# ai-forever/Kandinsky-2

Hardware: NVIDIA H100
Metric: unet_denoising_steps_per_sec (higher is better)
Workload: dtype f16

## Files before the change

kandinsky-2_b200/csrc/k2_api.cu:

```cuda
#include <stdio.h>
#include <stdlib.h>
#include <string.h>

#include <algorithm>
#include <atomic>
#include <mutex>

#include "../../include/k2b200.h"
#include "k2_internal.h"

namespace k2 {

static thread_local std::string g_err;
static std::atomic<long long> g_launches{0};
static int g_force_bn = 0;
static int g_force_split = 0;
static int g_pdl = 0;


void set_error(const std::string& msg) { g_err = msg; }
int fail(const std::string& msg) {
  g_err = msg;
  return -1;
}
void count_launch(int n) { g_launches.fetch_add(n, std::memory_order_relaxed); }

bool pdl_enabled() { return g_pdl != 0; }
static int g_conv_epi_sets = 1;
static int g_gn_bps = 0;
int gn_apply_blocks_per_sm() { return g_gn_bps; }

int num_sms() {
  static int n = 0;
  if (n == 0) {
    int dev = 0;
    cudaGetDevice(&dev);
    cudaDeviceGetAttribute(&n, cudaDevAttrMultiProcessorCount, dev);
    if (n <= 0) n = 132;
  }
  return n;
}

typedef CUresult (*EncodeTiledFn)(CUtensorMap*, CUtensorMapDataType, cuuint32_t, void*, const cuuint64_t*,
                                  const cuuint64_t*, const cuuint32_t*, const cuuint32_t*,
                                  CUtensorMapInterleave, CUtensorMapSwizzle, CUtensorMapL2promotion,
                                  CUtensorMapFloatOOBfill);

static EncodeTiledFn get_encode_fn() {
  static EncodeTiledFn fn = nullptr;
  static std::once_flag once;
  std::call_once(once, [] {
    void* p = nullptr;
    cudaDriverEntryPointQueryResult qres;
    cudaError_t e = cudaGetDriverEntryPoint("cuTensorMapEncodeTiled", &p, cudaEnableDefault, &qres);
    if (e == cudaSuccess && qres == cudaDriverEntryPointSuccess) fn = reinterpret_cast<EncodeTiledFn>(p);
  });
  return fn;
}

int encode_tmap_f16(CUtensorMap* out, const void* base, int rank, const uint64_t* dims,
                    const uint64_t* strides_bytes, const uint32_t* box) {
  EncodeTiledFn fn = get_encode_fn();
  if (!fn) return fail("cuTensorMapEncodeTiled unavailable (no CUDA driver)");
  cuuint64_t gdim[5];
  cuuint64_t gstr[4];
  cuuint32_t bx[5];
  cuuint32_t es[5];
  for (int i = 0; i < rank; ++i) {
    gdim[i] = dims[i];
    bx[i] = box[i];
    es[i] = 1;
  }
  for (int i = 0; i + 1 < rank; ++i) gstr[i] = strides_bytes[i];
  CUresult r = fn(out, CU_TENSOR_MAP_DATA_TYPE_FLOAT16, static_cast<cuuint32_t>(rank), const_cast<void*>(base),
                  gdim, gstr, bx, es, CU_TENSOR_MAP_INTERLEAVE_NONE, CU_TENSOR_MAP_SWIZZLE_128B,
                  CU_TENSOR_MAP_L2_PROMOTION_L2_256B, CU_TENSOR_MAP_FLOAT_OOB_FILL_NONE);
  if (r != CUDA_SUCCESS) {
    char buf[256];
    snprintf(buf, sizeof buf,
             "cuTensorMapEncodeTiled failed (%d): rank %d dims %llu %llu %llu %llu box %u %u %u %u base %p",
             static_cast<int>(r), rank, (unsigned long long)dims[0], (unsigned long long)(rank > 1 ? dims[1] : 0),
             (unsigned long long)(rank > 2 ? dims[2] : 0), (unsigned long long)(rank > 3 ? dims[3] : 0), box[0],
             rank > 1 ? box[1] : 0, rank > 2 ? box[2] : 0, rank > 3 ? box[3] : 0, base);
    return fail(buf);
  }
  return 0;
}

static void choose_tile(int NB, int H, int W, int& TN, int& TH, int& TW, bool single_image_only = false) {
  long long best_tiles[2] = {-1, -1};
  int bn[2] = {1, 1}, bw[2] = {1, 1}, bh[2] = {1, 1};
  const int wmax = W < 128 ? W : 128;
  for (int tw = 1; tw <= wmax; ++tw) {
    const long long tiles_w = (W + tw - 1) / tw;
    for (int tn = 1; tn <= NB && tn * tw <= 128; ++tn) {
      int thmax = 128 / (tw * tn);
      if (thmax > H) thmax = H;
      if (thmax < 1) continue;
      const long long tiles_h = (H + thmax - 1) / thmax;
      const int th = static_cast<int>((H + tiles_h - 1) / tiles_h);
      const long long tiles = tiles_h * tiles_w * ((NB + tn - 1) / tn);
      for (int k = (tn == 1 ? 0 : 1); k < 2; ++k) {
        bool better = best_tiles[k] < 0 || tiles < best_tiles[k];
        if (!better && tiles == best_tiles[k]) {
          if (tn != bn[k]) {
            better = tn < bn[k];
          } else {
            const int d_new = tw > th ? tw - th : th - tw;
            const int d_old = bw[k] > bh[k] ? bw[k] - bh[k] : bh[k] - bw[k];
            better = (d_new < d_old) || (d_new == d_old && tw > bw[k]);
          }
        }
        if (better) {
          best_tiles[k] = tiles;
          bn[k] = tn;
          bw[k] = tw;
          bh[k] = th;
        }
      }
    }
  }
  const int k = (!single_image_only && best_tiles[1] * 100 <= best_tiles[0] * 85) ? 1 : 0;
  TN = bn[k];
  TW = bw[k];
  TH = bh[k];
}


struct ConvPlan {
  int TN, TH, TW, tiles_w, tiles_h, tiles_n, m_tiles;
  int m_tiles_phase;
  int BN, splits;
  int fuse_stats, row_groups;
  int es;
};

static void plan_conv(int NB, int H, int W, bool any9, int kchunks, int Cout, int out_mode, bool has_workspace,
                      long long workspace_bytes, bool want_gn, ConvPlan& pl, const int* cfg = nullptr, bool up2 = false,
                      bool w_batched = false) {
  const int g_force_bn = (cfg && cfg[0]) ? cfg[0] : k2::g_force_bn;
  const int g_force_split = (cfg && cfg[2]) ? cfg[2] : k2::g_force_split;
  pl.es = (cfg && cfg[3]) ? cfg[3] : k2::g_conv_epi_sets;
  choose_tile(NB, H, W, pl.TN, pl.TH, pl.TW, w_batched);
  pl.tiles_w = (W + pl.TW - 1) / pl.TW;
  pl.tiles_h = (H + pl.TH - 1) / pl.TH;
  pl.tiles_n = (NB + pl.TN - 1) / pl.TN;
  pl.m_tiles = pl.tiles_w * pl.tiles_h * pl.tiles_n;
  pl.m_tiles_phase = pl.m_tiles;

  int BN = g_force_bn;
  int splits = 1;
  const long long M_total = static_cast<long long>(NB) * H * W;
  const bool can_split = !up2 && !w_batched && has_workspace && out_mode == 0 && Cout % 8 == 0;
  auto split_ok = [&](int sp) {
    if (sp == 1) return true;
    const int kps = (kchunks + sp - 1) / sp;
    return can_split && kps >= 8 && (sp - 1) * kps < kchunks &&
           static_cast<long long>(sp) * M_total * Cout * 4 <= workspace_bytes;
  };
  auto model = [&](int bn, int sp) {
    const long long nt = (Cout + bn - 1) / bn;
    const long long units = static_cast<long long>(pl.m_tiles) * nt * sp * (up2 ? 4 : 1);
    const long long slots = num_sms();
    const long long waves = (units + slots - 1) / slots;
    const long long kps = (kchunks + sp - 1) / sp;
    long long cost = waves * (kps * (4LL * bn + 60) + 2000);
    if (sp > 1) cost += 4000 + (static_cast<long long>(sp) + 1) * M_total * Cout * 4 / 1800;
    return cost;
  };
  if (BN == 0) {
    if (Cout <= 16) BN = 16;
    else if (Cout <= 64) BN = 64;
    else if (Cout <= 128) BN = 128;
    else BN = 0;
  }
  {
    const int cand[3] = {256, 192, 128};
    long long best = -1;
    int best_bn = BN ? BN : 256, best_sp = 1;
    for (int ci = 0; ci < 3; ++ci) {
      const int bn = BN ? BN : cand[ci];
      if (BN && ci > 0) break;
      for (int sp = 1; sp <= 8; ++sp) {
        if (g_force_split > 0 && sp != g_force_split) continue;
        if (!split_ok(sp)) continue;
        const long long c = model(bn, sp);
        if (best < 0 || c < best) {
          best = c;
          best_bn = bn;
          best_sp = sp;
        }
      }
    }
    BN = best_bn;
    splits = best_sp;
  }
  pl.BN = BN;
  pl.splits = splits;

  pl.fuse_stats = 0;
  pl.row_groups = 0;
  if (want_gn && out_mode == 0 && Cout % 8 == 0) {
    if (splits == 1 && BN >= 64 && Cout % 64 == 0 && (pl.TN == 1 || pl.TH * pl.TW == 16)) {
      pl.fuse_stats = 1;
      pl.row_groups = ((pl.TN == 1) ? pl.m_tiles : NB * pl.tiles_h * pl.tiles_w) * (up2 ? 4 : 1);
    } else if (splits > 1 && (static_cast<long long>(H) * W) % 16 == 0) {
      pl.fuse_stats = 2;
      pl.row_groups = static_cast<int>(M_total / 16);
    }
  }
}

static void plan_to_info(const ConvPlan& pl, int* info) {
  if (!info) return;
  info[0] = pl.BN; info[1] = 0;
  info[2] = pl.splits; info[3] = pl.m_tiles; info[4] = pl.TN;
  info[5] = pl.fuse_stats; info[6] = pl.row_groups;
}

}

using namespace k2;

extern "C" {

const char* k2_last_error(void) { return g_err.c_str(); }
int k2_version(void) { return 100; }
long long k2_launch_count(void) { return g_launches.load(); }
void k2_reset_launch_count(void) { g_launches.store(0); }
int k2_set_tuning(int key, int value) {
  if (key == 0) {
    g_force_bn = value;
    return 0;
  }
  if (key == 1) {
    g_force_split = value;
    return 0;
  }
  if (key == 2) {
    if (value == 2) return fail("k2_set_tuning: no CTA-pair conv kernel on sm_90");
    return 0;
  }
  if (key == 4) {
    g_pdl = value;
    return 0;
  }
  if (key == 10) {
    g_conv_epi_sets = (value == 2) ? 2 : 1;
    return 0;
  }
  if (key == 11) {
    g_gn_bps = value;
    return 0;
  }
  if (key == 9) {
    return 0;
  }

  return fail("k2_set_tuning: unknown key");
}

int k2_conv_gemm(const K2ConvSrc* srcs, int nsrc, int NB, int H, int W, const void* w_packed, int w_rows,
                 int Ktot, int ldw, int Cout, const float* bias, const void* residual, int ldr, void* out, int ldo,
                 int out_mode, void* workspace, long long workspace_bytes, float* gn_partial, int* info,
                 k2_stream_t stream) {
  return k2_conv_gemm_cfg(srcs, nsrc, NB, H, W, w_packed, w_rows, Ktot, ldw, Cout, bias, residual, ldr, out, ldo, out_mode,
                          workspace, workspace_bytes, gn_partial, info, nullptr, 0, stream);
}

int k2_conv_gemm_cfg(const K2ConvSrc* srcs, int nsrc, int NB, int H, int W, const void* w_packed, int w_rows,
                     int Ktot, int ldw, int Cout, const float* bias, const void* residual, int ldr, void* out, int ldo,
                     int out_mode, void* workspace, long long workspace_bytes, float* gn_partial, int* info,
                     const int* cfg, long long w_batch_stride, k2_stream_t stream) {
  K2_REQUIRE(w_batch_stride >= 0 && w_batch_stride % 8 == 0, "conv_gemm_cfg: w_batch_stride must be a multiple of 8 elements");
  K2_REQUIRE(out_mode == 0 || out_mode == 1, "conv_gemm: out_mode must be 0 (fp16 rows) or 1 (fp32 NCHW)");
  K2_REQUIRE(out_mode == 0 || residual == nullptr, "conv_gemm: out_mode 1 (fp32 NCHW) takes no residual");
  const bool w_batched = w_batch_stride > 0;
  if (cfg) {
    K2_REQUIRE(cfg[0] == 0 || cfg[0] == 16 || cfg[0] == 64 || cfg[0] == 128 || cfg[0] == 192 || cfg[0] == 256,
               "conv_gemm_cfg: N tile must be 0, 16, 64, 128, 192 or 256");
    K2_REQUIRE(cfg[1] >= 0 && cfg[1] <= 2 && cfg[2] >= 0 && cfg[2] <= 8 && cfg[3] >= 0 && cfg[3] <= 2,
               "conv_gemm_cfg: pair mode in 0..2, splits in 0..8, epilogue sets in 0..2");
    K2_REQUIRE(cfg[1] != 2, "conv_gemm_cfg: no CTA-pair conv kernel on sm_90");
  }
  K2_REQUIRE(nsrc >= 1 && nsrc <= 3, "conv_gemm: 1..3 sources");
  K2_REQUIRE((reinterpret_cast<uintptr_t>(gn_partial) & 7) == 0, "conv_gemm: gn_partial must be 8-byte aligned");
  K2_REQUIRE(NB > 0 && H > 0 && W > 0 && Cout > 0, "conv_gemm: bad geometry");
  K2_REQUIRE(w_rows >= Cout, "conv_gemm: w_rows < Cout");
  K2_REQUIRE(Ktot % 64 == 0, "conv_gemm: Ktot must be a multiple of 64");
  if (ldw == 0) ldw = Ktot;
  K2_REQUIRE(ldw >= Ktot && ldw % 8 == 0 && (reinterpret_cast<uintptr_t>(w_packed) & 15) == 0,
             "conv_gemm: weight row stride / alignment");
  ConvGemmParams p;
  memset(&p, 0, sizeof p);
  p.NB = NB;
  p.H = H;
  p.W = W;
  bool any9 = false;
  int kchunks = 0;
  const bool up2 = srcs[0].taps == 4;
  if (up2) {
    K2_REQUIRE(nsrc == 1 && out_mode == 0 && residual == nullptr && H % 2 == 0 && W % 2 == 0,
               "conv_gemm: a taps == 4 source (3x3 conv over its nearest-2x upsampling) must be the only source, with fp16 "
               "output, no residual and even output H, W");
    H /= 2;
    W /= 2;
    p.H = H;
    p.W = W;
  }
  for (int s = 0; s < nsrc; ++s) {
    const K2ConvSrc& src = srcs[s];
    K2_REQUIRE(src.taps == 9 || src.taps == 1 || (s == 0 && src.taps == 4), "conv_gemm: taps must be 9 or 1 (or 4: up2)");
    K2_REQUIRE(src.C > 0 && src.C % 8 == 0 && src.ld % 8 == 0 && src.ld >= src.C, "conv_gemm: bad source C/ld");
    K2_REQUIRE((reinterpret_cast<uintptr_t>(src.ptr) & 15) == 0, "conv_gemm: source not 16B aligned");
    any9 = any9 || src.taps == 9;
    p.seg_taps[s] = src.taps;
    p.seg_kchunks[s] = (src.C + 63) / 64;
    kchunks += src.taps * p.seg_kchunks[s];
  }
  K2_REQUIRE(kchunks * 64 * (up2 ? 4 : 1) == Ktot,
             "conv_gemm: Ktot does not match the sources (taps * ceil(C/64)*64 summed; x4 phases for a taps == 4 source)");
  p.num_k_chunks = kchunks;

  ConvPlan pl;
  plan_conv(NB, H, W, any9 || up2, kchunks, Cout, out_mode, workspace != nullptr, workspace_bytes, gn_partial != nullptr, pl,
            cfg, up2, w_batched);
  K2_REQUIRE(!w_batched || (!up2 && pl.TN == 1), "conv_gemm_cfg: batched weights need single-image tiles");
  p.w_batched = w_batched ? 1 : 0;
  plan_to_info(pl, info);
  p.TN = pl.TN;
  p.TH = pl.TH;
  p.TW = pl.TW;
  p.tiles_w = pl.tiles_w;
  p.tiles_h = pl.tiles_h;
  p.tiles_n = pl.tiles_n;
  p.m_tiles = up2 ? 4 * pl.m_tiles_phase : pl.m_tiles;
  p.m_tiles_phase = pl.m_tiles_phase;
  p.up2 = up2 ? 1 : 0;
  p.a_box_bytes = static_cast<uint32_t>(p.TN * p.TH * p.TW * 128);
  for (int s = 0; s < nsrc; ++s) {
    const K2ConvSrc& src = srcs[s];
    uint64_t dims[4] = {static_cast<uint64_t>(src.C), static_cast<uint64_t>(W), static_cast<uint64_t>(H),
                        static_cast<uint64_t>(NB)};
    uint64_t str[3] = {static_cast<uint64_t>(src.ld) * 2, static_cast<uint64_t>(src.ld) * 2 * W,
                       static_cast<uint64_t>(src.ld) * 2 * W * H};
    uint32_t box[4] = {64, static_cast<uint32_t>(p.TW), static_cast<uint32_t>(p.TH), static_cast<uint32_t>(p.TN)};
    if (encode_tmap_f16(&p.tmA[s], src.ptr, 4, dims, str, box)) return -1;
  }
  const int BN = pl.BN, splits = pl.splits, fuse_stats = pl.fuse_stats;
  p.splits = splits;
  p.k_per_split = (kchunks + splits - 1) / splits;
  p.M_total = static_cast<long long>(NB) * H * W * (up2 ? 4 : 1);
  p.ws = reinterpret_cast<float*>(workspace);
  p.n_tiles = (Cout + BN - 1) / BN;
  p.Cout = Cout;
  {
    uint64_t dims[3] = {static_cast<uint64_t>(Ktot), static_cast<uint64_t>(w_rows), static_cast<uint64_t>(w_batched ? NB : 1)};
    uint64_t str[2] = {static_cast<uint64_t>(ldw) * 2,
                       (w_batched ? static_cast<uint64_t>(w_batch_stride) : static_cast<uint64_t>(ldw) * w_rows) * 2};
    uint32_t box[3] = {64, static_cast<uint32_t>(BN), 1};
    if (encode_tmap_f16(&p.tmB, w_packed, 3, dims, str, box)) return -1;
  }
  p.bias = bias;
  p.residual = reinterpret_cast<const __half*>(residual);
  p.ldr = ldr;
  p.out = out;
  p.ldo = ldo;
  p.out_mode = (splits > 1) ? 2 : out_mode;
  p.gn_part = (fuse_stats == 1) ? reinterpret_cast<float2*>(gn_partial) : nullptr;
  p.gn_mode = (fuse_stats == 1) ? (p.TN == 1 ? 1 : 2) : 0;
  if (out_mode == 0) {
    K2_REQUIRE(ldo % 8 == 0 && (reinterpret_cast<uintptr_t>(out) & 15) == 0, "conv_gemm: out alignment");
    if (residual)
      K2_REQUIRE(ldr % 8 == 0 && (reinterpret_cast<uintptr_t>(residual) & 15) == 0, "conv_gemm: residual alignment");
  }
  int rc = launch_conv_gemm(p, BN, pl.es, static_cast<cudaStream_t>(stream));
  if (rc == 0) g_launches.fetch_add(1, std::memory_order_relaxed);
  if (rc == 0 && splits > 1) {
    rc = launch_splitk_finalize(p.ws, splits, p.M_total, Cout, bias, p.residual, ldr, reinterpret_cast<__half*>(out), ldo,
                                fuse_stats == 2 ? reinterpret_cast<float2*>(gn_partial) : nullptr,
                                static_cast<cudaStream_t>(stream));
    if (rc == 0) g_launches.fetch_add(1, std::memory_order_relaxed);
  }
  return rc;
}

int k2_conv_plan(int NB, int H, int W, int taps, int Ktot, int Cout, int out_mode, long long workspace_bytes,
                 int want_gn_partial, int* info) {
  K2_REQUIRE(NB > 0 && H > 0 && W > 0 && Cout > 0 && info, "conv_plan: bad arguments");
  K2_REQUIRE(Ktot > 0 && Ktot % 64 == 0, "conv_plan: Ktot must be a positive multiple of 64");
  ConvPlan pl;
  plan_conv(NB, H, W, taps == 9, Ktot / 64, Cout, out_mode, workspace_bytes > 0, workspace_bytes, want_gn_partial != 0, pl);
  plan_to_info(pl, info);
  return 0;
}

}
```

kandinsky-2_b200/csrc/k2_common.cuh:

```cuda
#pragma once
#include <cuda.h>
#include <cuda_fp16.h>
#include <cuda_runtime.h>
#include <stdint.h>
#include <stdio.h>

namespace k2 {

__device__ __forceinline__ uint32_t smem_u32(const void* p) {
  return static_cast<uint32_t>(__cvta_generic_to_shared(p));
}

__device__ __forceinline__ uint32_t lane_id() { return threadIdx.x & 31; }

__device__ __forceinline__ bool elect_one() {
  uint32_t pred = 0;
  asm volatile(
      "{\n"
      ".reg .b32 rx;\n"
      ".reg .pred px;\n"
      "elect.sync rx|px, 0xffffffff;\n"
      "selp.b32 %0, 1, 0, px;\n"
      "}\n"
      : "=r"(pred));
  return pred != 0;
}

__device__ __forceinline__ void mbar_init(uint64_t* bar, uint32_t count) {
  asm volatile("mbarrier.init.shared::cta.b64 [%0], %1;" ::"r"(smem_u32(bar)), "r"(count));
}
__device__ __forceinline__ void fence_barrier_init() {
  asm volatile("fence.mbarrier_init.release.cluster;" ::: "memory");
}
__device__ __forceinline__ void mbar_arrive_expect_tx(uint64_t* bar, uint32_t bytes) {
  asm volatile("mbarrier.arrive.expect_tx.shared::cta.b64 _, [%0], %1;" ::"r"(smem_u32(bar)),
               "r"(bytes)
               : "memory");
}
__device__ __forceinline__ void mbar_arrive(uint64_t* bar) {
  asm volatile("mbarrier.arrive.shared::cta.b64 _, [%0];" ::"r"(smem_u32(bar)) : "memory");
}
__device__ __forceinline__ bool mbar_try_wait(uint64_t* bar, uint32_t parity) {
  uint32_t ok;
  asm volatile(
      "{\n"
      ".reg .pred p;\n"
      "mbarrier.try_wait.parity.shared::cta.b64 p, [%1], %2;\n"
      "selp.b32 %0, 1, 0, p;\n"
      "}\n"
      : "=r"(ok)
      : "r"(smem_u32(bar)), "r"(parity)
      : "memory");
  return ok != 0;
}
__device__ __forceinline__ void mbar_wait(uint64_t* bar, uint32_t parity) {
  if (mbar_try_wait(bar, parity)) return;
  long long t0 = clock64();
  while (!mbar_try_wait(bar, parity)) {
    if (clock64() - t0 > 4000000000LL) {
      printf("k2b200: mbarrier wait timeout (block %d,%d,%d thread %d)\n", blockIdx.x, blockIdx.y,
             blockIdx.z, threadIdx.x);
      __trap();
    }
  }
}

__device__ __forceinline__ void mbar_wait_lean(uint64_t* bar, uint32_t parity) {
  if (mbar_try_wait(bar, parity)) return;
  long long t0 = clock64();
  while (!mbar_try_wait(bar, parity)) {
    if (clock64() - t0 > 4000000000LL) __trap();
  }
}

__device__ __forceinline__ void fence_proxy_async_smem() {
  asm volatile("fence.proxy.async.shared::cta;" ::: "memory");
}

__device__ __forceinline__ void tma_prefetch_desc(const CUtensorMap* tm) {
  asm volatile("prefetch.tensormap [%0];" ::"l"(reinterpret_cast<uint64_t>(tm)) : "memory");
}
__device__ __forceinline__ void tma_load_2d(void* dst, const CUtensorMap* tm, uint64_t* bar, int c0,
                                            int c1) {
  asm volatile(
      "cp.async.bulk.tensor.2d.shared::cluster.global.mbarrier::complete_tx::bytes [%0], [%1, {%3, "
      "%4}], [%2];"
      ::"r"(smem_u32(dst)),
      "l"(reinterpret_cast<uint64_t>(tm)), "r"(smem_u32(bar)), "r"(c0), "r"(c1)
      : "memory");
}
__device__ __forceinline__ void tma_load_3d(void* dst, const CUtensorMap* tm, uint64_t* bar, int c0,
                                            int c1, int c2) {
  asm volatile(
      "cp.async.bulk.tensor.3d.shared::cluster.global.mbarrier::complete_tx::bytes [%0], [%1, {%3, "
      "%4, %5}], [%2];"
      ::"r"(smem_u32(dst)),
      "l"(reinterpret_cast<uint64_t>(tm)), "r"(smem_u32(bar)), "r"(c0), "r"(c1), "r"(c2)
      : "memory");
}
__device__ __forceinline__ void tma_load_4d(void* dst, const CUtensorMap* tm, uint64_t* bar, int c0,
                                            int c1, int c2, int c3) {
  asm volatile(
      "cp.async.bulk.tensor.4d.shared::cluster.global.mbarrier::complete_tx::bytes [%0], [%1, {%3, "
      "%4, %5, %6}], [%2];"
      ::"r"(smem_u32(dst)),
      "l"(reinterpret_cast<uint64_t>(tm)), "r"(smem_u32(bar)), "r"(c0), "r"(c1), "r"(c2), "r"(c3)
      : "memory");
}

__device__ __forceinline__ uint64_t make_wgmma_desc(uint32_t smem_addr) {
  uint64_t d = 0;
  d |= static_cast<uint64_t>((smem_addr & 0x3FFFF) >> 4);
  d |= static_cast<uint64_t>(1) << 16;
  d |= static_cast<uint64_t>(1024 >> 4) << 32;
  d |= static_cast<uint64_t>(1) << 62;
  return d;
}
__device__ __forceinline__ void wgmma_fence() { asm volatile("wgmma.fence.sync.aligned;" ::: "memory"); }
__device__ __forceinline__ void wgmma_commit() { asm volatile("wgmma.commit_group.sync.aligned;" ::: "memory"); }
template <int N>
__device__ __forceinline__ void wgmma_wait() {
  asm volatile("wgmma.wait_group.sync.aligned %0;" ::"n"(N) : "memory");
}
__device__ __forceinline__ void wgmma_m64n16k16(float (&d)[8], uint64_t adesc, uint64_t bdesc, uint32_t accumulate) {
  asm volatile(
      "{\n"
      ".reg .pred p;\n"
      "setp.ne.b32 p, %10, 0;\n"
      "wgmma.mma_async.sync.aligned.m64n16k16.f32.f16.f16 "
      "{%0, %1, %2, %3, %4, %5, %6, %7}, %8, %9, p, 1, 1, 0, 0;\n"
      "}\n"
      : "+f"(d[0]), "+f"(d[1]), "+f"(d[2]), "+f"(d[3]), "+f"(d[4]), "+f"(d[5]), "+f"(d[6]), "+f"(d[7])
      : "l"(adesc), "l"(bdesc), "r"(accumulate));
}

__device__ __forceinline__ void wgmma_m64n64k16(float (&d)[32], uint64_t adesc, uint64_t bdesc, uint32_t accumulate) {
  asm volatile(
      "{\n"
      ".reg .pred p;\n"
      "setp.ne.b32 p, %34, 0;\n"
      "wgmma.mma_async.sync.aligned.m64n64k16.f32.f16.f16 "
      "{%0, %1, %2, %3, %4, %5, %6, %7, %8, %9, %10, %11, %12, %13, %14, %15, %16, %17, %18, %19, %20, %21, %22, %23, %24, %25, %26, %27, %28, %29, %30, %31}, %32, %33, p, 1, 1, 0, 0;\n"
      "}\n"
      : "+f"(d[0]), "+f"(d[1]), "+f"(d[2]), "+f"(d[3]), "+f"(d[4]), "+f"(d[5]), "+f"(d[6]), "+f"(d[7]), "+f"(d[8]), "+f"(d[9]), "+f"(d[10]), "+f"(d[11]), "+f"(d[12]), "+f"(d[13]), "+f"(d[14]), "+f"(d[15]), "+f"(d[16]), "+f"(d[17]), "+f"(d[18]), "+f"(d[19]), "+f"(d[20]), "+f"(d[21]), "+f"(d[22]), "+f"(d[23]), "+f"(d[24]), "+f"(d[25]), "+f"(d[26]), "+f"(d[27]), "+f"(d[28]), "+f"(d[29]), "+f"(d[30]), "+f"(d[31])
      : "l"(adesc), "l"(bdesc), "r"(accumulate));
}

#define K2_WGMMA_D8(o)                                                                                                  \
  "+f"(d[(o)]), "+f"(d[(o) + 1]), "+f"(d[(o) + 2]), "+f"(d[(o) + 3]), "+f"(d[(o) + 4]), "+f"(d[(o) + 5]), "+f"(d[(o) + 6]), \
      "+f"(d[(o) + 7])
#define K2_WGMMA_D32(o) K2_WGMMA_D8(o), K2_WGMMA_D8((o) + 8), K2_WGMMA_D8((o) + 16), K2_WGMMA_D8((o) + 24)

__device__ __forceinline__ void wgmma_m64n128k16(float (&d)[64], uint64_t adesc, uint64_t bdesc, uint32_t accumulate) {
  asm volatile(
      "{\n"
      ".reg .pred p;\n"
      "setp.ne.b32 p, %66, 0;\n"
      "wgmma.mma_async.sync.aligned.m64n128k16.f32.f16.f16 {"
      "%0, %1, %2, %3, %4, %5, %6, %7, %8, %9, %10, %11, %12, %13, %14, %15, "
      "%16, %17, %18, %19, %20, %21, %22, %23, %24, %25, %26, %27, %28, %29, %30, %31, "
      "%32, %33, %34, %35, %36, %37, %38, %39, %40, %41, %42, %43, %44, %45, %46, %47, "
      "%48, %49, %50, %51, %52, %53, %54, %55, %56, %57, %58, %59, %60, %61, %62, %63"
      "}, %64, %65, p, 1, 1, 0, 0;\n"
      "}\n"
      : K2_WGMMA_D32(0), K2_WGMMA_D32(32)
      : "l"(adesc), "l"(bdesc), "r"(accumulate));
}

__device__ __forceinline__ void wgmma_m64n192k16(float (&d)[96], uint64_t adesc, uint64_t bdesc, uint32_t accumulate) {
  asm volatile(
      "{\n"
      ".reg .pred p;\n"
      "setp.ne.b32 p, %98, 0;\n"
      "wgmma.mma_async.sync.aligned.m64n192k16.f32.f16.f16 {"
      "%0, %1, %2, %3, %4, %5, %6, %7, %8, %9, %10, %11, %12, %13, %14, %15, "
      "%16, %17, %18, %19, %20, %21, %22, %23, %24, %25, %26, %27, %28, %29, %30, %31, "
      "%32, %33, %34, %35, %36, %37, %38, %39, %40, %41, %42, %43, %44, %45, %46, %47, "
      "%48, %49, %50, %51, %52, %53, %54, %55, %56, %57, %58, %59, %60, %61, %62, %63, "
      "%64, %65, %66, %67, %68, %69, %70, %71, %72, %73, %74, %75, %76, %77, %78, %79, "
      "%80, %81, %82, %83, %84, %85, %86, %87, %88, %89, %90, %91, %92, %93, %94, %95"
      "}, %96, %97, p, 1, 1, 0, 0;\n"
      "}\n"
      : K2_WGMMA_D32(0), K2_WGMMA_D32(32), K2_WGMMA_D32(64)
      : "l"(adesc), "l"(bdesc), "r"(accumulate));
}

__device__ __forceinline__ void wgmma_m64n256k16(float (&d)[128], uint64_t adesc, uint64_t bdesc, uint32_t accumulate) {
  asm volatile(
      "{\n"
      ".reg .pred p;\n"
      "setp.ne.b32 p, %130, 0;\n"
      "wgmma.mma_async.sync.aligned.m64n256k16.f32.f16.f16 {"
      "%0, %1, %2, %3, %4, %5, %6, %7, %8, %9, %10, %11, %12, %13, %14, %15, "
      "%16, %17, %18, %19, %20, %21, %22, %23, %24, %25, %26, %27, %28, %29, %30, %31, "
      "%32, %33, %34, %35, %36, %37, %38, %39, %40, %41, %42, %43, %44, %45, %46, %47, "
      "%48, %49, %50, %51, %52, %53, %54, %55, %56, %57, %58, %59, %60, %61, %62, %63, "
      "%64, %65, %66, %67, %68, %69, %70, %71, %72, %73, %74, %75, %76, %77, %78, %79, "
      "%80, %81, %82, %83, %84, %85, %86, %87, %88, %89, %90, %91, %92, %93, %94, %95, "
      "%96, %97, %98, %99, %100, %101, %102, %103, %104, %105, %106, %107, %108, %109, %110, %111, "
      "%112, %113, %114, %115, %116, %117, %118, %119, %120, %121, %122, %123, %124, %125, %126, %127"
      "}, %128, %129, p, 1, 1, 0, 0;\n"
      "}\n"
      : K2_WGMMA_D32(0), K2_WGMMA_D32(32), K2_WGMMA_D32(64), K2_WGMMA_D32(96)
      : "l"(adesc), "l"(bdesc), "r"(accumulate));
}
__device__ __forceinline__ uint64_t make_wgmma_desc_mn(uint32_t smem_addr) {
  uint64_t d = 0;
  d |= static_cast<uint64_t>((smem_addr & 0x3FFFF) >> 4);
  d |= static_cast<uint64_t>(1) << 16;
  d |= static_cast<uint64_t>(1024 >> 4) << 32;
  d |= static_cast<uint64_t>(1) << 62;
  return d;
}

__device__ __forceinline__ void wgmma_m64n64k16_rs_tb(float (&d)[32], const uint32_t (&a)[4], uint64_t bdesc) {
  asm volatile(
      "{\n"
      "wgmma.mma_async.sync.aligned.m64n64k16.f32.f16.f16 {"
      "%0, %1, %2, %3, %4, %5, %6, %7, %8, %9, %10, %11, %12, %13, %14, %15, "
      "%16, %17, %18, %19, %20, %21, %22, %23, %24, %25, %26, %27, %28, %29, %30, %31"
      "}, {%32, %33, %34, %35}, %36, 1, 1, 1, 1;\n"
      "}\n"
      : K2_WGMMA_D32(0)
      : "r"(a[0]), "r"(a[1]), "r"(a[2]), "r"(a[3]), "l"(bdesc));
}
#undef K2_WGMMA_D32
#undef K2_WGMMA_D8

__device__ __forceinline__ void reg_fence(float& r) { asm volatile("" : "+f"(r)::"memory"); }

template <int R>
__device__ __forceinline__ void setmaxnreg_dec() {
  asm volatile("setmaxnreg.dec.sync.aligned.u32 %0;" ::"n"(R));
}
template <int R>
__device__ __forceinline__ void setmaxnreg_inc() {
  asm volatile("setmaxnreg.inc.sync.aligned.u32 %0;" ::"n"(R));
}

__device__ __forceinline__ void mma_16816(float (&d)[4], const uint32_t (&a)[4], uint32_t b0, uint32_t b1) {
  asm volatile(
      "mma.sync.aligned.m16n8k16.row.col.f32.f16.f16.f32 {%0, %1, %2, %3}, {%4, %5, %6, %7}, {%8, %9}, "
      "{%0, %1, %2, %3};"
      : "+f"(d[0]), "+f"(d[1]), "+f"(d[2]), "+f"(d[3])
      : "r"(a[0]), "r"(a[1]), "r"(a[2]), "r"(a[3]), "r"(b0), "r"(b1));
}
__device__ __forceinline__ void ldmatrix_x4(uint32_t (&r)[4], uint32_t saddr) {
  asm volatile("ldmatrix.sync.aligned.m8n8.x4.shared.b16 {%0, %1, %2, %3}, [%4];"
               : "=r"(r[0]), "=r"(r[1]), "=r"(r[2]), "=r"(r[3])
               : "r"(saddr));
}
__device__ __forceinline__ void ldmatrix_x4_trans(uint32_t (&r)[4], uint32_t saddr) {
  asm volatile("ldmatrix.sync.aligned.m8n8.x4.trans.shared.b16 {%0, %1, %2, %3}, [%4];"
               : "=r"(r[0]), "=r"(r[1]), "=r"(r[2]), "=r"(r[3])
               : "r"(saddr));
}
__device__ __forceinline__ void cp_async_16(uint32_t saddr, const void* gptr, int src_bytes) {
  asm volatile("cp.async.cg.shared.global [%0], [%1], 16, %2;" ::"r"(saddr), "l"(gptr), "r"(src_bytes) : "memory");
}
__device__ __forceinline__ void cp_async_commit() { asm volatile("cp.async.commit_group;" ::: "memory"); }
template <int N>
__device__ __forceinline__ void cp_async_wait() {
  asm volatile("cp.async.wait_group %0;" ::"n"(N) : "memory");
}

__device__ __forceinline__ void sts_v4(uint32_t saddr, uint32_t a, uint32_t b, uint32_t c, uint32_t d) {
  asm volatile("st.shared.v4.b32 [%0], {%1, %2, %3, %4};" ::"r"(saddr), "r"(a), "r"(b), "r"(c), "r"(d) : "memory");
}
__device__ __forceinline__ uint4 lds_v4(uint32_t saddr) {
  uint4 v;
  asm volatile("ld.shared.v4.b32 {%0, %1, %2, %3}, [%4];" : "=r"(v.x), "=r"(v.y), "=r"(v.z), "=r"(v.w) : "r"(saddr) : "memory");
  return v;
}
__device__ __forceinline__ uint32_t lds_u32(uint32_t saddr) {
  uint32_t v;
  asm volatile("ld.shared.b32 %0, [%1];" : "=r"(v) : "r"(saddr) : "memory");
  return v;
}
__device__ __forceinline__ void named_bar_sync(int id, int count) {
  asm volatile("bar.sync %0, %1;" ::"r"(id), "r"(count) : "memory");
}
__device__ __forceinline__ void named_bar_arrive(int id, int count) {
  asm volatile("bar.arrive %0, %1;" ::"r"(id), "r"(count) : "memory");
}
__device__ __forceinline__ void pdl_wait() { asm volatile("griddepcontrol.wait;" ::: "memory"); }
__device__ __forceinline__ void pdl_launch() { asm volatile("griddepcontrol.launch_dependents;" ::: "memory"); }

__device__ __forceinline__ float silu_f(float x) {
  float e, r;
  asm("ex2.approx.ftz.f32 %0, %1;" : "=f"(e) : "f"(-1.44269504088896341f * x));
  asm("rcp.approx.ftz.f32 %0, %1;" : "=f"(r) : "f"(1.f + e));
  return x * r;
}

}
```

kandinsky-2_b200/csrc/k2_conv_gemm.cu:

```cuda
#include <stdio.h>

#include "k2_common.cuh"
#include "k2_internal.h"

namespace k2 {

namespace {

constexpr int BM = 128;
constexpr int BK = 64;
constexpr int A_STAGE_BYTES = BM * BK * 2;
constexpr int ACC_PAD = 4;

constexpr int EPI_STAGE_FLOATS = 32 * 33;
constexpr int EPI_BYTES = 4 * EPI_STAGE_FLOATS * 4 + 4 * 256 * 4;
constexpr int SMEM_LIMIT = 227 * 1024;

template <int BN, int ES>
struct Cfg {
  static constexpr int B_STAGE_BYTES = BN * BK * 2;
  static constexpr int STAGE_BYTES = A_STAGE_BYTES + B_STAGE_BYTES;
  static constexpr int BNC = (BN < 64) ? BN : (ES == 2 ? 128 : 64);
  static_assert(ES == 1 || BN % 128 == 0, "two epilogue sets need N tiles of 128 or 256");
  static constexpr int ACC_BYTES = BM * (BNC + ACC_PAD) * 4;
  static constexpr int BAR_BYTES = 256;
  static constexpr int FIXED = ACC_BYTES + ES * EPI_BYTES + BAR_BYTES + 1024;
  static constexpr int STAGES = (SMEM_LIMIT - FIXED) / STAGE_BYTES > 6 ? 6 : (SMEM_LIMIT - FIXED) / STAGE_BYTES;
  static constexpr int SMEM_BYTES = STAGES * STAGE_BYTES + FIXED;
  static_assert(STAGES >= 2, "conv_gemm: shared memory does not hold two pipeline stages");
};

__device__ __forceinline__ void decode_m_tile(const ConvGemmParams& p, int m_idx, int& n0, int& y0,
                                              int& x0, int& phase) {
  phase = 0;
  if (p.up2) {
    phase = m_idx / p.m_tiles_phase;
    m_idx -= phase * p.m_tiles_phase;
  }
  int tw_i = m_idx % p.tiles_w;
  int t = m_idx / p.tiles_w;
  int th_i = t % p.tiles_h;
  int tn_i = t / p.tiles_h;
  x0 = tw_i * p.TW;
  y0 = th_i * p.TH;
  n0 = tn_i * p.TN;
}

template <int N>
__device__ __forceinline__ void acc_ld(const float* src, uint32_t (&r)[N]) {
#pragma unroll
  for (int v = 0; v < N / 4; ++v) {
    const float4 t = *reinterpret_cast<const float4*>(src + 4 * v);
    r[4 * v] = __float_as_uint(t.x);
    r[4 * v + 1] = __float_as_uint(t.y);
    r[4 * v + 2] = __float_as_uint(t.z);
    r[4 * v + 3] = __float_as_uint(t.w);
  }
}

template <int BN, int ES>
__device__ __forceinline__ void epilogue_tile(const ConvGemmParams& p, const float* acc, int ew, int lane, int n0, int y0,
                                              int x0, int cbase, int split, int m_idx, float* stat_smem, int es_arg,
                                              int phase) {
  const int es = (ES == 1) ? 0 : es_arg;
  const int row = ew * 32 + lane;
  const int thw = p.TH * p.TW;
  constexpr int CH = (BN >= 32) ? 32 : 16;
  const float* arow = acc + row * (BN + ACC_PAD);
      const int tn = row / thw;
      const int rem = row - tn * thw;
      const int th = rem / p.TW;
      const int tw = rem - th * p.TW;
      const int n = n0 + tn, y = y0 + th, x = x0 + tw;
      const bool valid = (tn < p.TN) && (n < p.NB) && (y < p.H) && (x < p.W);
      const long long out_row = p.up2 ? (static_cast<long long>(n) * (2 * p.H) + (2 * y + (phase >> 1))) * (2 * p.W) + (2 * x + (phase & 1))
                                      : (static_cast<long long>(n) * p.H + y) * p.W + x;
      const int m_in = p.up2 ? m_idx - phase * p.m_tiles_phase : m_idx;
      auto part_index = [&](long long base) { return p.up2 ? base * 4 + phase : base; };
      if constexpr (BN % 64 == 0) {
        if ((p.out_mode == 0 && p.Cout % 64 == 0) || (p.out_mode == 2 && p.Cout % 32 == 0)) {
          const uint32_t stage = smem_u32(stat_smem + (es * 4 + ew) * EPI_STAGE_FLOATS);
          float* bsm = stat_smem + 4 * ES * EPI_STAGE_FLOATS + (es * 4 + ew) * 256;
          const int my_pix = valid ? static_cast<int>(out_row) : -1;
          const int sub = lane >> 3, piece = lane & 7;
          int pix[8];
#pragma unroll
          for (int i = 0; i < 8; ++i) pix[i] = __shfl_sync(0xffffffffu, my_pix, i * 4 + sub);
          const uint32_t own = stage + lane * 128;
          if (p.out_mode == 2) {
            float* wsb = p.ws + static_cast<long long>(split) * p.M_total * p.Cout;
#pragma unroll 1
            for (int j = 0; j < BN / 32; ++j) {
              const int col0 = cbase + j * 32;
              if (col0 >= p.Cout) break;
              if constexpr (ES > 1) {
                if ((j % ES) != es) continue;
              }
              uint32_t r[32];
              acc_ld(arow + j * 32, r);
#pragma unroll
              for (int v = 0; v < 8; ++v)
                sts_v4(own + ((v ^ (lane & 7)) << 4), r[v * 4], r[v * 4 + 1], r[v * 4 + 2], r[v * 4 + 3]);
              __syncwarp();
#pragma unroll
              for (int i = 0; i < 8; ++i) {
                const int rr = i * 4 + sub;
                const uint4 v4 = lds_v4(stage + rr * 128 + ((piece ^ (rr & 7)) << 4));
                if (pix[i] >= 0)
                  *reinterpret_cast<uint4*>(wsb + static_cast<long long>(pix[i]) * p.Cout + col0 + piece * 4) = v4;
              }
              __syncwarp();
            }
            return;
          }
          constexpr int NP = BN / 64;
          if (p.bias) {
#pragma unroll
            for (int c = lane; c < BN; c += 32) bsm[c] = (cbase + c < p.Cout) ? __ldg(p.bias + cbase + c) : 0.f;
            __syncwarp();
          }
          __half* outb = reinterpret_cast<__half*>(p.out);
          float4 st[NP];
          uint4 rpre[8];
          auto load_res = [&](int jp) {
            const int c0 = cbase + jp * 64;
#pragma unroll
            for (int i = 0; i < 8; ++i) {
              rpre[i] = make_uint4(0u, 0u, 0u, 0u);
              if (pix[i] >= 0 && c0 < p.Cout)
                rpre[i] = *reinterpret_cast<const uint4*>(p.residual + static_cast<long long>(pix[i]) * p.ldr + c0 + piece * 8);
            }
          };
          if constexpr (ES == 1) {
            if (p.residual) load_res(0);
          }
#pragma unroll
          for (int jp = 0; jp < NP; ++jp) {
            const int col0 = cbase + jp * 64;
            st[jp] = make_float4(0.f, 0.f, 0.f, 0.f);
            if (col0 < p.Cout && (ES == 1 || (jp % ES) == es)) {
              if constexpr (ES > 1) {
                if (p.residual) load_res(jp);
              }
              if (p.residual) {
#pragma unroll
                for (int i = 0; i < 8; ++i) {
                  const int rr = i * 4 + sub;
                  sts_v4(stage + rr * 128 + ((piece ^ (rr & 7)) << 4), rpre[i].x, rpre[i].y, rpre[i].z, rpre[i].w);
                }
                __syncwarp();
              }
              if constexpr (ES == 1) {
                if (p.residual && jp + 1 < NP) load_res(jp + 1);
              }
#pragma unroll
              for (int v = 0; v < 8; ++v) {
                uint32_t r[8];
                acc_ld(arow + jp * 64 + v * 8, r);
                float f[8];
#pragma unroll
                for (int e = 0; e < 8; ++e) f[e] = __uint_as_float(r[e]);
                if (p.bias) {
                  const float4 b0 = *reinterpret_cast<const float4*>(bsm + jp * 64 + v * 8);
                  const float4 b1 = *reinterpret_cast<const float4*>(bsm + jp * 64 + v * 8 + 4);
                  f[0] += b0.x; f[1] += b0.y; f[2] += b0.z; f[3] += b0.w;
                  f[4] += b1.x; f[5] += b1.y; f[6] += b1.z; f[7] += b1.w;
                }
                const uint32_t slot = own + ((v ^ (lane & 7)) << 4);
                if (p.residual) {
                  const uint4 rv = lds_v4(slot);
                  const __half2* rh = reinterpret_cast<const __half2*>(&rv);
#pragma unroll
                  for (int e = 0; e < 4; ++e) {
                    const float2 t = __half22float2(rh[e]);
                    f[2 * e] += t.x;
                    f[2 * e + 1] += t.y;
                  }
                }
                uint32_t o[4];
#pragma unroll
                for (int e = 0; e < 4; ++e) {
                  const __half2 hh = __floats2half2_rn(f[2 * e], f[2 * e + 1]);
                  o[e] = valid ? *reinterpret_cast<const uint32_t*>(&hh) : 0u;
                }
                sts_v4(slot, o[0], o[1], o[2], o[3]);
              }
              __syncwarp();
#pragma unroll
              for (int i = 0; i < 8; ++i) {
                const int rr = i * 4 + sub;
                const uint4 v4 = lds_v4(stage + rr * 128 + ((piece ^ (rr & 7)) << 4));
                if (pix[i] >= 0)
                  *reinterpret_cast<uint4*>(outb + static_cast<long long>(pix[i]) * p.ldo + col0 + piece * 8) = v4;
              }
              if (p.gn_part) {
                float4 h0 = make_float4(0.f, 0.f, 0.f, 0.f), h1 = make_float4(0.f, 0.f, 0.f, 0.f);
#pragma unroll
                for (int rr = 0; rr < 32; ++rr) {
                  const uint32_t w = lds_u32(stage + rr * 128 + (((lane >> 2) ^ (rr & 7)) << 4) + ((lane & 3) << 2));
                  const float2 t = __half22float2(*reinterpret_cast<const __half2*>(&w));
                  float4& hacc = (rr < 16) ? h0 : h1;
                  hacc.x += t.x;
                  hacc.y = fmaf(t.x, t.x, hacc.y);
                  hacc.z += t.y;
                  hacc.w = fmaf(t.y, t.y, hacc.w);
                }
                if (p.gn_mode == 2) {
                  const int per = p.tiles_h * p.tiles_w;
                  const int sp = m_in % per;
                  const int img = n0 + 2 * ew;
                  if (2 * ew < p.TN && img < p.NB)
                    *reinterpret_cast<float4*>(p.gn_part + part_index(static_cast<long long>(img) * per + sp) * p.Cout + col0 + 2 * lane) = h0;
                  if (2 * ew + 1 < p.TN && img + 1 < p.NB)
                    *reinterpret_cast<float4*>(p.gn_part + part_index(static_cast<long long>(img + 1) * per + sp) * p.Cout + col0 + 2 * lane) = h1;
                } else {
                  st[jp] = make_float4(h0.x + h1.x, h0.y + h1.y, h0.z + h1.z, h0.w + h1.w);
                }
              }
              __syncwarp();
            }
          }
          if (p.gn_part && p.gn_mode == 1) {
            if constexpr (ES == 1) {
              float4* mine = reinterpret_cast<float4*>(stat_smem + ew * EPI_STAGE_FLOATS);
#pragma unroll
              for (int jp = 0; jp < NP; ++jp) mine[jp * 32 + lane] = st[jp];
              named_bar_sync(1, 128);
              if (ew < NP) {
                const int col0 = cbase + ew * 64;
                if (col0 < p.Cout) {
                  float4 acc = make_float4(0.f, 0.f, 0.f, 0.f);
#pragma unroll
                  for (int w = 0; w < 4; ++w) {
                    const float4 t = reinterpret_cast<const float4*>(stat_smem + w * EPI_STAGE_FLOATS)[ew * 32 + lane];
                    acc.x += t.x; acc.y += t.y; acc.z += t.z; acc.w += t.w;
                  }
                  *reinterpret_cast<float4*>(p.gn_part + part_index(m_in) * p.Cout + col0 + 2 * lane) = acc;
                }
              }
              named_bar_sync(1, 128);
            } else {
              float4* mine = reinterpret_cast<float4*>(stat_smem + (es * 4 + ew) * EPI_STAGE_FLOATS);
#pragma unroll
              for (int jp = 0; jp < NP; ++jp) mine[jp * 32 + lane] = st[jp];
              named_bar_sync(1 + es, 128);
              const int jp_f = es + ew * ES;
              if (jp_f < NP) {
                const int col0 = cbase + jp_f * 64;
                if (col0 < p.Cout) {
                  float4 acc = make_float4(0.f, 0.f, 0.f, 0.f);
#pragma unroll
                  for (int w = 0; w < 4; ++w) {
                    const float4 t =
                        reinterpret_cast<const float4*>(stat_smem + (es * 4 + w) * EPI_STAGE_FLOATS)[jp_f * 32 + lane];
                    acc.x += t.x; acc.y += t.y; acc.z += t.z; acc.w += t.w;
                  }
                  *reinterpret_cast<float4*>(p.gn_part + part_index(m_in) * p.Cout + col0 + 2 * lane) = acc;
                }
              }
              named_bar_sync(1 + es, 128);
            }
          }
          return;
        }
      }
#pragma unroll 1
      for (int j = 0; j < BN / CH; ++j) {
        uint32_t r[CH];
        acc_ld(arow + j * CH, r);
        const int col0 = cbase + j * CH;
        if (valid && col0 < p.Cout) {
          if (p.out_mode == 2) {
            float* w = p.ws + (static_cast<long long>(split) * p.M_total + out_row) * p.Cout + col0;
            if (col0 + CH <= p.Cout) {
#pragma unroll
              for (int v = 0; v < CH / 4; ++v)
                *reinterpret_cast<uint4*>(w + v * 4) = make_uint4(r[v * 4], r[v * 4 + 1], r[v * 4 + 2], r[v * 4 + 3]);
            } else {
#pragma unroll
              for (int e = 0; e < CH; ++e)
                if (col0 + e < p.Cout) w[e] = __uint_as_float(r[e]);
            }
          } else if (p.out_mode == 0) {
            __half* orow = reinterpret_cast<__half*>(p.out) + out_row * p.ldo + col0;
            const __half* rrow = p.residual ? p.residual + out_row * p.ldr + col0 : nullptr;
            if (col0 + CH <= p.Cout) {
#pragma unroll
              for (int v = 0; v < CH / 8; ++v) {
                float f[8];
#pragma unroll
                for (int e = 0; e < 8; ++e) {
                  f[e] = __uint_as_float(r[v * 8 + e]);
                  if (p.bias) f[e] += __ldg(p.bias + col0 + v * 8 + e);
                }
                if (rrow) {
                  uint4 rv = *reinterpret_cast<const uint4*>(rrow + v * 8);
                  const __half2* rh = reinterpret_cast<const __half2*>(&rv);
#pragma unroll
                  for (int e = 0; e < 4; ++e) {
                    float2 t = __half22float2(rh[e]);
                    f[2 * e] += t.x;
                    f[2 * e + 1] += t.y;
                  }
                }
                uint4 ov;
                __half2* oh = reinterpret_cast<__half2*>(&ov);
#pragma unroll
                for (int e = 0; e < 4; ++e) oh[e] = __floats2half2_rn(f[2 * e], f[2 * e + 1]);
                *reinterpret_cast<uint4*>(orow + v * 8) = ov;
              }
            } else {
#pragma unroll
              for (int e = 0; e < CH; ++e) {
                if (col0 + e < p.Cout) {
                  float f = __uint_as_float(r[e]);
                  if (p.bias) f += __ldg(p.bias + col0 + e);
                  if (rrow) f += __half2float(rrow[e]);
                  orow[e] = __float2half_rn(f);
                }
              }
            }
          } else {
            float* o = reinterpret_cast<float*>(p.out);
#pragma unroll
            for (int e = 0; e < CH; ++e) {
              if (col0 + e < p.Cout) {
                float f = __uint_as_float(r[e]);
                if (p.bias) f += __ldg(p.bias + col0 + e);
                o[((static_cast<long long>(n) * p.Cout + (col0 + e)) * p.H + y) * p.W + x] = f;
              }
            }
          }
        }
      }
}


template <int BN, int ES>
__global__ void __launch_bounds__(384, 1) conv_gemm_kernel(const __grid_constant__ ConvGemmParams p) {
  using C = Cfg<BN, ES>;
  constexpr int BNC = C::BNC;
  constexpr int NA = BN / 2;
  extern __shared__ uint8_t smem_raw[];
  uint8_t* smem = reinterpret_cast<uint8_t*>((reinterpret_cast<uintptr_t>(smem_raw) + 1023) &
                                             ~static_cast<uintptr_t>(1023));
  float* acc_smem = reinterpret_cast<float*>(smem + C::STAGES * C::STAGE_BYTES);
  float* stat_smem = reinterpret_cast<float*>(smem + C::STAGES * C::STAGE_BYTES + C::ACC_BYTES);
  uint64_t* full_bar = reinterpret_cast<uint64_t*>(smem + C::STAGES * C::STAGE_BYTES + C::ACC_BYTES + ES * EPI_BYTES);
  uint64_t* empty_bar = full_bar + C::STAGES;

  const int warp_idx = threadIdx.x >> 5;
  const int lane = threadIdx.x & 31;
  const int wg = warp_idx >> 2;

  if (threadIdx.x == 0) {
    tma_prefetch_desc(&p.tmB);
    for (int s = 0; s < 3; ++s)
      if (p.seg_taps[s]) tma_prefetch_desc(&p.tmA[s]);
    for (int i = 0; i < C::STAGES; ++i) {
      mbar_init(&full_bar[i], 1);
      mbar_init(&empty_bar[i], 8);
    }
    fence_barrier_init();
  }
  __syncthreads();
  pdl_wait();
  pdl_launch();

  const int total_tiles = p.m_tiles * p.n_tiles * p.splits;

  if (wg == 0) {
    setmaxnreg_dec<40>();
    if (warp_idx == 0 && elect_one()) {
      int stage = 0;
      uint32_t ring_phase = 0;
      const uint32_t tx_bytes = p.a_box_bytes + C::B_STAGE_BYTES;
      for (int tile = blockIdx.x; tile < total_tiles; tile += gridDim.x) {
        const int n_idx = tile % p.n_tiles;
        const int m_idx = (tile / p.n_tiles) % p.m_tiles;
        const int split = tile / (p.m_tiles * p.n_tiles);
        int n0, y0, x0, phase;
        decode_m_tile(p, m_idx, n0, y0, x0, phase);
        const int kb = phase * p.num_k_chunks;
        const int k0 = split * p.k_per_split;
        const int k1 = min(p.num_k_chunks, k0 + p.k_per_split);
        int s = 0, rem = k0;
        while (rem >= p.seg_taps[s] * p.seg_kchunks[s]) {
          rem -= p.seg_taps[s] * p.seg_kchunks[s];
          ++s;
        }
        int tap = rem / p.seg_kchunks[s];
        int c = rem - tap * p.seg_kchunks[s];
        for (int kc = k0; kc < k1; ++kc) {
          const int taps = p.seg_taps[s];
          const int dy = (taps == 9) ? (tap / 3 - 1) : (taps == 4 ? (tap >> 1) + (phase >> 1) - 1 : 0);
          const int dx = (taps == 9) ? (tap % 3 - 1) : (taps == 4 ? (tap & 1) + (phase & 1) - 1 : 0);
          mbar_wait_lean(&empty_bar[stage], ring_phase ^ 1);
          uint8_t* sA = smem + stage * C::STAGE_BYTES;
          uint8_t* sB = sA + A_STAGE_BYTES;
          mbar_arrive_expect_tx(&full_bar[stage], tx_bytes);
          tma_load_4d(sA, &p.tmA[s], &full_bar[stage], c * BK, x0 + dx, y0 + dy, n0);
          tma_load_3d(sB, &p.tmB, &full_bar[stage], (kb + kc) * BK, n_idx * BN, p.w_batched ? n0 : 0);
          if (++stage == C::STAGES) {
            stage = 0;
            ring_phase ^= 1;
          }
          if (++c == p.seg_kchunks[s]) {
            c = 0;
            if (++tap == taps) {
              tap = 0;
              ++s;
            }
          }
        }
      }
    }
  } else {
    setmaxnreg_inc<232>();
    const int g = wg - 1;
    const int w = warp_idx & 3;
    int stage = 0;
    uint32_t phase = 0;
    for (int tile = blockIdx.x; tile < total_tiles; tile += gridDim.x) {
      const int n_idx = tile % p.n_tiles;
      const int m_idx = (tile / p.n_tiles) % p.m_tiles;
      const int split = tile / (p.m_tiles * p.n_tiles);
      const int nk = min(p.num_k_chunks, (split + 1) * p.k_per_split) - split * p.k_per_split;
      float acc[NA];
#pragma unroll
      for (int i = 0; i < NA; ++i) acc[i] = 0.f;
      int prev_stage = -1;
      for (int kc = 0; kc < nk; ++kc) {
        mbar_wait_lean(&full_bar[stage], phase);
        const uint32_t a_addr = smem_u32(smem + stage * C::STAGE_BYTES) + g * (64 * 128);
        const uint32_t b_addr = smem_u32(smem + stage * C::STAGE_BYTES + A_STAGE_BYTES);
        wgmma_fence();
#pragma unroll
        for (int k = 0; k < BK / 16; ++k) {
          const uint64_t adesc = make_wgmma_desc(a_addr) + static_cast<uint64_t>(k * 2);
          const uint64_t bdesc = make_wgmma_desc(b_addr) + static_cast<uint64_t>(k * 2);
          if constexpr (BN == 256) {
            wgmma_m64n256k16(acc, adesc, bdesc, 1u);
          } else if constexpr (BN == 192) {
            wgmma_m64n192k16(acc, adesc, bdesc, 1u);
          } else if constexpr (BN == 128) {
            wgmma_m64n128k16(acc, adesc, bdesc, 1u);
          } else if constexpr (BN == 64) {
            wgmma_m64n64k16(acc, adesc, bdesc, 1u);
          } else {
            static_assert(BN == 16, "conv_gemm: N tile without a wgmma shape");
            wgmma_m64n16k16(acc, adesc, bdesc, 1u);
          }
        }
        wgmma_commit();
        wgmma_wait<1>();
        if (prev_stage >= 0 && lane == 0) mbar_arrive(&empty_bar[prev_stage]);
        prev_stage = stage;
        if (++stage == C::STAGES) {
          stage = 0;
          phase ^= 1;
        }
      }
      wgmma_wait<0>();
      if (prev_stage >= 0 && lane == 0) mbar_arrive(&empty_bar[prev_stage]);

      int n0, y0, x0, mphase;
      decode_m_tile(p, m_idx, n0, y0, x0, mphase);
      const int r0 = 64 * g + 16 * w + (lane >> 2);
      const int cq = 2 * (lane & 3);
#pragma unroll
      for (int pass = 0; pass < BN / BNC; ++pass) {
        named_bar_sync(3, 256);
#pragma unroll
        for (int i = 0; i < NA; i += 2) {
          if ((8 * (i >> 2)) / BNC != pass) continue;
          const int row = r0 + 8 * ((i >> 1) & 1);
          const int col = 8 * (i >> 2) - pass * BNC + cq;
          *reinterpret_cast<float2*>(acc_smem + row * (BNC + ACC_PAD) + col) = make_float2(acc[i], acc[i + 1]);
        }
        named_bar_sync(3, 256);
        if (ES == 2 || g == 0)
          epilogue_tile<BNC, ES>(p, acc_smem, w, lane, n0, y0, x0, n_idx * BN + pass * BNC, split, m_idx, stat_smem, g,
                                 mphase);
      }
    }
  }
}

__global__ void __launch_bounds__(256) splitk_finalize_kernel(const float* __restrict__ ws, int splits, long long M,
                                                              int Cout, const float* __restrict__ bias,
                                                              const __half* __restrict__ residual, int ldr,
                                                              __half* __restrict__ out, int ldo, float2* __restrict__ gn_part) {
  __shared__ float red[8][32][17];
  const int vx = threadIdx.x & 31, ry = threadIdx.x >> 5;
  const int c0 = (blockIdx.y * 32 + vx) * 8;
  const long long rg = blockIdx.x;
  pdl_wait();
  pdl_launch();
  float st[16];
#pragma unroll
  for (int e = 0; e < 16; ++e) st[e] = 0.f;
  if (c0 < Cout) {
    float bv[8];
#pragma unroll
    for (int e = 0; e < 8; ++e) bv[e] = bias ? __ldg(bias + c0 + e) : 0.f;
#pragma unroll
    for (int rr = 0; rr < 2; ++rr) {
      const long long m = rg * 16 + ry + rr * 8;
      if (m >= M) continue;
      float f[8];
#pragma unroll
      for (int e = 0; e < 8; ++e) f[e] = bv[e];
      for (int s = 0; s < splits; ++s) {
        const float4* w = reinterpret_cast<const float4*>(ws + (static_cast<long long>(s) * M + m) * Cout + c0);
        const float4 a = __ldcs(w), b = __ldcs(w + 1);
        f[0] += a.x; f[1] += a.y; f[2] += a.z; f[3] += a.w; f[4] += b.x; f[5] += b.y; f[6] += b.z; f[7] += b.w;
      }
      if (residual) {
        const uint4 rv = __ldg(reinterpret_cast<const uint4*>(residual + m * ldr + c0));
        const __half2* rh = reinterpret_cast<const __half2*>(&rv);
#pragma unroll
        for (int e = 0; e < 4; ++e) {
          const float2 t = __half22float2(rh[e]);
          f[2 * e] += t.x;
          f[2 * e + 1] += t.y;
        }
      }
      uint4 ov;
      __half2* oh = reinterpret_cast<__half2*>(&ov);
#pragma unroll
      for (int e = 0; e < 4; ++e) {
        oh[e] = __floats2half2_rn(f[2 * e], f[2 * e + 1]);
        const float2 t = __half22float2(oh[e]);
        st[2 * e] += t.x;
        st[2 * e + 1] += t.y;
        st[8 + 2 * e] = fmaf(t.x, t.x, st[8 + 2 * e]);
        st[8 + 2 * e + 1] = fmaf(t.y, t.y, st[8 + 2 * e + 1]);
      }
      *reinterpret_cast<uint4*>(out + m * ldo + c0) = ov;
    }
  }
  if (gn_part == nullptr) return;
#pragma unroll
  for (int e = 0; e < 16; ++e) red[ry][vx][e] = st[e];
  __syncthreads();
  const int vx2 = threadIdx.x >> 3, e2 = threadIdx.x & 7;
  const int c = (blockIdx.y * 32 + vx2) * 8 + e2;
  if (c < Cout) {
    float s1 = 0.f, s2 = 0.f;
#pragma unroll
    for (int q = 0; q < 8; ++q) {
      s1 += red[q][vx2][e2];
      s2 += red[q][vx2][8 + e2];
    }
    gn_part[rg * Cout + c] = make_float2(s1, s2);
  }
}


template <int BN, int ES>
int launch_bn(const ConvGemmParams& p, cudaStream_t stream) {
  using C = Cfg<BN, ES>;
  static bool attr_set = false;
  if (!attr_set) {
    K2_CHECK_CUDA(cudaFuncSetAttribute(conv_gemm_kernel<BN, ES>, cudaFuncAttributeMaxDynamicSharedMemorySize,
                                       C::SMEM_BYTES));
    attr_set = true;
  }
  int total = p.m_tiles * p.n_tiles * p.splits;
  int grid = total < num_sms() ? total : num_sms();
  K2_CHECK_CUDA(launch_k(conv_gemm_kernel<BN, ES>, dim3(grid), dim3(384), C::SMEM_BYTES, stream, p));
  return 0;
}

}

int launch_splitk_finalize(const float* ws, int splits, long long M, int Cout, const float* bias, const __half* residual,
                           int ldr, __half* out, int ldo, float2* gn_part, cudaStream_t stream) {
  dim3 grid(static_cast<unsigned int>((M + 15) / 16), (Cout / 8 + 31) / 32);
  K2_CHECK_CUDA(launch_k(splitk_finalize_kernel, grid, dim3(256), 0, stream, ws, splits, M, Cout, bias, residual, ldr, out, ldo,
                         gn_part));
  return 0;
}

int launch_conv_gemm(const ConvGemmParams& p, int BN, int epilogue_sets, cudaStream_t stream) {
  if (epilogue_sets == 2) {
    switch (BN) {
      case 128: return launch_bn<128, 2>(p, stream);
      case 256: return launch_bn<256, 2>(p, stream);
      default: break;
    }
  }
  switch (BN) {
    case 16: return launch_bn<16, 1>(p, stream);
    case 64: return launch_bn<64, 1>(p, stream);
    case 128: return launch_bn<128, 1>(p, stream);
    case 192: return launch_bn<192, 1>(p, stream);
    case 256: return launch_bn<256, 1>(p, stream);
    default: return fail("conv_gemm: unsupported BN");
  }
}

}
```

kandinsky-2_b200/csrc/k2_internal.h:

```cpp
#pragma once
#include <cuda.h>
#include <cuda_fp16.h>
#include <cuda_runtime.h>
#include <stdint.h>

#include <string>

namespace k2 {

void set_error(const std::string& msg);
int fail(const std::string& msg);
#define K2_CHECK_CUDA(expr)                                                                 \
  do {                                                                                      \
    cudaError_t _e = (expr);                                                                \
    if (_e != cudaSuccess)                                                                  \
      return ::k2::fail(std::string(#expr) + ": " + cudaGetErrorString(_e));                \
  } while (0)
#define K2_REQUIRE(cond, msg)                                  \
  do {                                                         \
    if (!(cond)) return ::k2::fail(std::string("k2b200: ") + (msg)); \
  } while (0)

inline bool aligned16(const void* p) { return (reinterpret_cast<uintptr_t>(p) & 15) == 0; }

int num_sms();
bool pdl_enabled();

template <typename... KArgs, typename... Args>
inline cudaError_t launch_k(void (*kernel)(KArgs...), dim3 grid, dim3 block, size_t smem, cudaStream_t stream,
                            Args&&... args) {
  cudaLaunchConfig_t cfg = {};
  cfg.gridDim = grid;
  cfg.blockDim = block;
  cfg.dynamicSmemBytes = smem;
  cfg.stream = stream;
  cudaLaunchAttribute attr[1];
  attr[0].id = cudaLaunchAttributeProgrammaticStreamSerialization;
  attr[0].val.programmaticStreamSerializationAllowed = 1;
  cfg.attrs = attr;
  cfg.numAttrs = pdl_enabled() ? 1 : 0;
  return cudaLaunchKernelEx(&cfg, kernel, static_cast<KArgs>(args)...);
}
void count_launch(int n = 1);

int encode_tmap_f16(CUtensorMap* out, const void* base, int rank, const uint64_t* dims,
                    const uint64_t* strides_bytes , const uint32_t* box);

struct ConvGemmParams {
  CUtensorMap tmA[3];
  CUtensorMap tmB;
  int w_batched;
  int seg_taps[3];
  int seg_kchunks[3];
  int num_k_chunks;
  int NB, H, W;
  int TN, TH, TW;
  int tiles_n, tiles_h, tiles_w;
  int m_tiles, n_tiles;
  int Cout;
  const float* bias;
  const __half* residual;
  int ldr;
  void* out;
  int ldo;
  int out_mode;
  uint32_t a_box_bytes;
  int splits;
  int k_per_split;
  float* ws;
  long long M_total;
  float2* gn_part;
  int gn_mode;
  int up2;
  int m_tiles_phase;
};
int launch_conv_gemm(const ConvGemmParams& p, int BN, int epilogue_sets, cudaStream_t stream);
int launch_splitk_finalize(const float* ws, int splits, long long M, int Cout, const float* bias, const __half* residual,
                           int ldr, __half* out, int ldo, float2* gn_part, cudaStream_t stream);

struct FlashParams {
  const __half* qkv;
  long long ldq;
  int hs, q_off, k_off, v_off;
  const __half* enc;
  long long lde;
  int ehs, ek_off, ev_off;
  int B, heads, T, Tc;
  __half* out;
  int ldo, ohs;
  float scale_log2e;
};
int gn_apply_blocks_per_sm();
int launch_attention(const FlashParams& p, int head_dim, cudaStream_t stream);

}
```

kandinsky-2_b200/kandinsky2/launch_plan.py:

```python
import gc
import os

import torch

from . import ops

FOLD_MAX_RG = int(os.environ.get("K2_GN_FOLD_MAX_RG", "18"))
TUNE = os.environ.get("K2_AUTOTUNE", "1") != "0"
FORK = os.environ.get("K2_FORK", "1") != "0"
TUNE_SMALL_M = int(os.environ.get("K2_TUNE_SMALL_M", "8192"))
_tune_cache = {}


def tune(key, run, m_rows=0):
    if not TUNE:
        return None
    key = (torch.cuda.current_device(), TUNE_SMALL_M) + key
    if key in _tune_cache:
        return _tune_cache[key]
    info = [0] * 7
    run(None, info)
    bn0, splits = info[0], info[2]
    cout = key[3]
    best = None
    if cout > 64:
        bns = [bn0] if splits > 1 else [bn for bn in (128, 192, 256) if bn - 64 < cout or bn == bn0]
        cands = [(bn0, 0, splits, 1)] + [(bn, 0, splits, es) for bn in bns for es in ((1,) if bn == 192 else (1, 2))
                                        if (bn, es) != (bn0, 1)]
        if 0 < m_rows <= TUNE_SMALL_M and splits == 1:
            for bn in (128, 192, 256):
                if bn - 64 >= cout:
                    continue
                for sp in (2, 3, 4):
                    probe = [0] * 7
                    try:
                        run((bn, 1, sp, 1), probe)
                    except Exception:
                        continue
                    if probe[0] == bn and probe[2] == sp:
                        cands.append((bn, 1, sp, 1))

        def timed(cfg, reps=6):
            run(cfg)
            evs = [torch.cuda.Event(enable_timing=True) for _ in range(reps + 1)]
            evs[0].record()
            for i in range(reps):
                run(cfg)
                evs[i + 1].record()
            torch.cuda.synchronize()
            return min(evs[i].elapsed_time(evs[i + 1]) for i in range(reps))

        t0 = tb = timed(cands[0])
        for cfg in cands[1:]:
            t = timed(cfg)
            if t < tb and t < 0.97 * t0:
                t = max(t, timed(cfg))
                if t < tb and t < 0.97 * t0:
                    best, tb = cfg, t
    _tune_cache[key] = best
    return best


class LaunchPlan:
    def __init__(self, dev, nb):
        self.dev = dev
        self.NB = nb
        self._parts = {}
        self._scratch = {}
        self.steps = []
        self.graph = None
        self._side_stream = None
        self._side_open = False
        self._serial = False

    def _tmp(self, slot, *shape, dtype=torch.float16):
        key = (slot, dtype) + tuple(shape)
        if key not in self._scratch:
            self._scratch[key] = torch.empty(*shape, device=self.dev, dtype=dtype)
        return self._scratch[key]

    def _new(self, *shape, dtype=torch.float16):
        return torch.empty(*shape, device=self.dev, dtype=dtype)

    def _add(self, fn, kind="misc", flops=0):
        fn()
        self.steps.append((fn, kind, flops))

    def _side(self, fn, kind="misc", flops=0):
        if not FORK:
            return self._add(fn, kind, flops)
        first = not self._side_open
        self._side_open = True

        def step():
            if self._serial:
                return fn()
            if self._side_stream is None:
                self._side_stream = torch.cuda.Stream(device=self.dev)
            if first:
                ev = torch.cuda.Event()
                ev.record()
                self._side_stream.wait_event(ev)
            with torch.cuda.stream(self._side_stream):
                fn()
        self._add(step, kind, flops)

    def _join(self):
        if not self._side_open:
            return
        self._side_open = False

        def step():
            if self._serial:
                return
            ev = torch.cuda.Event()
            ev.record(self._side_stream)
            torch.cuda.current_stream().wait_event(ev)
        self._add(step, "join", 0)

    def _conv(self, srcs, w, cout, out, flops, bias=None, residual=None, want_stats=True, part_slot=None, out_mode=0,
              geom=None, w_batch_stride=0, kind="conv_gemm"):
        part = None
        if want_stats and out_mode == 0:
            g = geom if geom is not None else tuple(out.shape[:3])
            n = ops.gn_part_floats(g[0], g[1], g[2], cout)
            part = self._tmp(part_slot, n, dtype=torch.float32) if part_slot else self._new(n, dtype=torch.float32)
        info = [0] * 7
        run = lambda cfg, info=None: ops.conv_gemm(srcs, w, cout, bias=bias, residual=residual, out=out, gn_part=part,
                                                   info=info, cfg=cfg, out_mode=out_mode, geom=geom,
                                                   w_batch_stride=w_batch_stride)
        key = ("conv", cout, tuple(out.shape), geom, tuple((t.shape[-1], taps) for t, taps in srcs), residual is not None,
               part is not None, out_mode, w_batch_stride > 0)
        cfg = tune(key, run, m_rows=out.shape[0] * out.shape[1] * out.shape[2] if out_mode == 0 and geom is None else 0)
        self._add(lambda: run(cfg, info), kind, flops)
        if part is not None and info[5]:
            self._parts[out.data_ptr()] = (part, info[6] // (geom[0] if geom is not None else out.shape[0]))
        else:
            self._parts.pop(out.data_ptr(), None)

    def _gemm(self, x, w, cout, out, flops, bias=None, residual=None):
        run = lambda cfg, info=None: ops.gemm_rows(x, w, cout, bias=bias, residual=residual, out=out, cfg=cfg, info=info)
        cfg = tune(("gemm", cout, tuple(x.shape), residual is not None), run, m_rows=x.shape[0] * x.shape[1])
        self._add(lambda: run(cfg), "conv_gemm", flops)
        self._parts.pop(out.data_ptr(), None)

    def _stats(self, a, b, eps):
        pa = self._parts.get(a.data_ptr())
        pb = self._parts.get(b.data_ptr()) if b is not None else None
        st = self._new(self.NB, 32, 2, dtype=torch.float32)
        HW = a.shape[1] * a.shape[2]
        if pa is not None and (b is None or pb is not None):
            c1 = b.shape[-1] if b is not None else 0
            self._add(lambda: ops.gn_finalize(pa[0], a.shape[-1], pb[0] if pb else None, c1, self.NB, pa[1], HW, st,
                                              rg1=pb[1] if pb else None, eps=eps), "gn_finalize")
        else:
            self._add(lambda: ops.gn_stats(a, b, stats=st, eps=eps), "gn_stats")
        return st

    def _norm(self, a, b, gamma, beta, y, film=None, act=1, resample=0, xres=None, eps=1e-5):
        pa = self._parts.get(a.data_ptr())
        pb = self._parts.get(b.data_ptr()) if b is not None else None
        have = pa is not None and (b is None or pb is not None)
        cpg = (a.shape[-1] + (b.shape[-1] if b is not None else 0)) // 32
        if have and cpg >= 2 and max(pa[1], pb[1] if pb else 0) <= FOLD_MAX_RG:
            self._add(lambda: ops.gn_apply_fold(a, b, pa[0], pa[1], pb[0] if pb else None, pb[1] if pb else 0, gamma, beta,
                                                film=film, act=act, resample=resample, y=y, xres=xres, eps=eps), "gn_apply")
            return
        st = self._stats(a, b, eps)
        self._add(lambda: ops.gn_apply(a, b, st, gamma, beta, film=film, act=act, resample=resample, y=y, xres=xres),
                  "gn_apply")

    def launch(self):
        for fn, _, _ in self.steps:
            fn()

    def _timed_pass(self):
        evs = []
        self._serial = True
        torch.cuda.synchronize()
        torch.cuda._sleep(int(4e7))
        for fn, kind, flops in self.steps:
            s = torch.cuda.Event(enable_timing=True)
            e = torch.cuda.Event(enable_timing=True)
            s.record()
            fn()
            e.record()
            evs.append((s, e))
        torch.cuda.synchronize()
        self._serial = False
        return [s.elapsed_time(e) for s, e in evs]

    def profile_detail(self, reps=3):
        acc = [0.0] * len(self.steps)
        for _ in range(reps):
            for i, ms in enumerate(self._timed_pass()):
                acc[i] += ms / reps
        return [(k, f, ms) for (_, k, f), ms in zip(self.steps, acc)]

    def profile(self, reps=3):
        agg = {}
        for kind, flops, ms in self.profile_detail(reps):
            if kind == "join":
                continue
            a = agg.setdefault(kind, dict(ms=0.0, launches=0, flops=0))
            a["ms"] += ms
            a["launches"] += 1
            a["flops"] += flops
        return agg

    def run(self, use_graph):
        if not use_graph:
            self.launch()
            return
        if self.graph is None:
            self.launch()
            torch.cuda.synchronize()
            self.graph = capture_graph(self.launch)
        self.graph.replay()


def capture_graph(launch):
    g = torch.cuda.CUDAGraph()
    enabled = gc.isenabled()
    gc.disable()
    try:
        with torch.cuda.graph(g):
            launch()
    finally:
        if enabled:
            gc.enable()
    return g
```

profiles/conv_layers.py:

```python
import argparse
import json
import os
import subprocess
import sys

ROOT = os.path.dirname(os.path.dirname(os.path.abspath(__file__)))
for p in (ROOT, os.path.join(ROOT, "kandinsky-2_b200")):
    if p not in sys.path:
        sys.path.insert(0, p)

import torch

B, H, W = 4, 96, 96


def _card():
    q = subprocess.run(["nvidia-smi", "--query-gpu=name,power.limit,clocks.max.sm", "--format=csv,noheader", "-i", "0"],
                       capture_output=True, text=True)
    return q.stdout.strip() or torch.cuda.get_device_name(0)


def _pad64(c):
    return (c + 63) // 64 * 64


def _layer(key, dev, g):
    from kandinsky2 import ops
    rnd = lambda *s: torch.randn(*s, device=dev, generator=g).half()
    kind, cout = key[0], key[1]
    if kind == "gemm":
        _, _, xshape, has_res = key
        x = rnd(*xshape)
        M, K = x.numel() // xshape[-1], xshape[-1]
        w = rnd(cout, K)
        bias = torch.randn(cout, device=dev, generator=g)
        res = rnd(*xshape[:-1], cout) if has_res else None
        out = torch.empty(*xshape[:-1], cout, device=dev, dtype=torch.float16)
        run = lambda cfg, info=None: ops.gemm_rows(x, w, cout, bias=bias, residual=res, out=out, cfg=cfg, info=info)
        return run, dict(M=M, N=cout, K=K, desc=f"gemm {M}x{K}->{cout}" + (" +res" if has_res else ""))
    _, _, oshape, geom, srcs_spec, has_res, has_part, out_mode, w_batched = key
    if w_batched:
        return None, None
    if geom is not None:
        NB, Ho, Wo = geom
    elif out_mode == 0:
        NB, Ho, Wo = oshape[:3]
    else:
        NB, Ho, Wo = oshape[0], oshape[2], oshape[3]
    up2 = srcs_spec[0][1] == 4
    Hs, Ws = (Ho // 2, Wo // 2) if up2 else (Ho, Wo)
    srcs = [(rnd(NB, Hs, Ws, c), taps) for c, taps in srcs_spec]
    K = sum(taps * _pad64(c) for c, taps in srcs_spec)
    w_rows = max(16, cout)
    w = rnd(w_rows, 4 * K if up2 else K)
    bias = torch.randn(cout, device=dev, generator=g)
    res = rnd(NB, Ho, Wo, cout) if has_res else None
    out = torch.empty(*oshape, device=dev, dtype=torch.float16 if out_mode == 0 else torch.float32)
    part = torch.zeros(ops.gn_part_floats(NB, Ho, Wo, cout), device=dev) if has_part else None
    run = lambda cfg, info=None: ops.conv_gemm(srcs, w, cout, bias=bias, residual=res, out=out, out_mode=out_mode, geom=geom,
                                               gn_part=part, cfg=cfg, info=info)
    desc = (f"{NB}x{Ho}x{Wo} " + "+".join(f"{c}{'x3x3' if t == 9 else ('up2' if t == 4 else 'x1x1')}" for c, t in srcs_spec)
            + f"->{cout}" + (" +res" if has_res else "") + (" fp32-nchw" if out_mode else ""))
    return run, dict(M=NB * Ho * Wo, N=cout, K=K, desc=desc)


def _time(run, cfg, min_ms):
    for _ in range(3):
        run(cfg)
    torch.cuda.synchronize()
    s, e = torch.cuda.Event(enable_timing=True), torch.cuda.Event(enable_timing=True)
    s.record()
    for _ in range(5):
        run(cfg)
    e.record()
    torch.cuda.synchronize()
    reps = max(10, int(min_ms / max(s.elapsed_time(e) / 5, 1e-3)) + 1)
    s.record()
    for _ in range(reps):
        run(cfg)
    e.record()
    torch.cuda.synchronize()
    return s.elapsed_time(e) / reps, reps


def main():
    ap = argparse.ArgumentParser()
    ap.add_argument("--out", default=None)
    ap.add_argument("--min-ms", type=float, default=50.0, help="timed window per configuration")
    ap.add_argument("--mma-n", default="tile", choices=["tile", "64"],
                    help="wgmma N of the build: one instruction per N tile, or m64n64k16 per 64 columns")
    args = ap.parse_args()
    if not torch.cuda.is_available():
        raise SystemExit("needs a CUDA sm_90 device")
    import bench
    from kandinsky2 import launch_plan, ops
    from kandinsky2.model.gaussian_diffusion import FusedStep, create_ddpm_v22
    dev = torch.device("cuda", 0)
    torch.cuda.set_device(dev)
    ops.set_tuning(4, 1)
    res = {"card": _card(), "torch": torch.__version__, "geometry": f"cfg-2: UNet batch {2 * B}, {H}x{W} latents",
           "mma_n": args.mma_n, "min_ms": args.min_ms}

    counts = {}
    tune = launch_plan.tune

    def counting_tune(key, run, m_rows=0):
        counts[key] = counts.get(key, 0) + 1
        return tune(key, run, m_rows=m_rows)
    launch_plan.tune = counting_tune
    model = bench.build_unet(dev)
    image_emb = torch.randn(2 * B, 1280, generator=torch.Generator().manual_seed(1234)).to(dev)
    step = FusedStep(model, B, H, W, dict(image_emb=image_emb), guidance_scale=4.0, cond_first=False, clip_range=2.0,
                     threshold_mode=0)
    launch_plan.tune = tune
    diffusion = create_ddpm_v22(50)
    coef, ts = diffusion._tables(dev)
    order = torch.arange(diffusion.num_timesteps - 1, -1, -1, device=dev)
    step.set_schedule(ts[order], coef[order], torch.randn(len(order), B, 4, H, W, device=dev))
    x = step.latent()
    x.copy_(torch.randn(B, 4, H, W, device=dev))
    step.advance(x)
    torch.cuda.synchronize()
    res["plan_conv_launches"] = sum(1 for _, kind, _ in step.plan.steps if kind == "conv_gemm")
    res["counted_conv_launches"] = sum(counts.values())

    g = torch.Generator(device=dev).manual_seed(7)
    layers = []
    for key, n in counts.items():
        run, shp = _layer(key, dev, g)
        if run is None:
            continue
        info = [0] * 7
        picked = launch_plan._tune_cache.get((dev.index, launch_plan.TUNE_SMALL_M) + key)
        run(picked, info)
        picked_cfg = [info[0], 0, info[2], (picked[3] if picked and picked[3] else 1)]
        cout = shp["N"]
        cfgs = []
        if cout > 64:
            cfgs = [(bn, 0, 1, es) for bn in (128, 192, 256) if bn - 64 < cout or bn == info[0]
                    for es in ((1,) if bn == 192 else (1, 2))]
        if tuple(picked_cfg) not in cfgs:
            cfgs.append(tuple(picked_cfg))
        rows = []
        for cfg in cfgs:
            info = [0] * 7
            run(cfg, info)
            bn, splits = info[0], info[2]
            ms, reps = _time(run, cfg, args.min_ms)
            flops = 2.0 * shp["M"] * cout * shp["K"]
            mma_n = bn if (args.mma_n == "tile" or bn < 64) else 64
            smem_bpf = (2048 + 32 * mma_n) / (2.0 * 64 * mma_n * 16)
            m_tiles = info[3] * (4 if "up2" in shp["desc"] else 1)
            chunks = m_tiles * ((cout + bn - 1) // bn) * (shp["K"] // 64)
            l2_bytes = chunks * (16384 + bn * 128)
            rows.append(dict(n_tile=bn, epilogue_sets=cfg[3], splits=splits, ms=round(ms, 5), reps=reps,
                             tflops=round(flops / (ms * 1e-3) / 1e12, 1),
                             smem_operand_bytes_per_flop=round(smem_bpf, 5),
                             l2_operand_bytes_per_flop=round(l2_bytes / flops, 5),
                             l2_operand_TBps=round(l2_bytes / (ms * 1e-3) / 1e12, 2)))
        pick = next((r for r in rows if [r["n_tile"], r["splits"], r["epilogue_sets"]] ==
                     [picked_cfg[0], picked_cfg[2], picked_cfg[3]]), rows[0])
        layers.append(dict(shape=shp["desc"], key=repr(key), launches_per_step=n, gemm_gflop=round(2e-9 * shp["M"] * cout * shp["K"], 3),
                           picked=dict(n_tile=picked_cfg[0], splits=picked_cfg[2], epilogue_sets=picked_cfg[3],
                                       tuned=picked is not None),
                           picked_ms=pick["ms"], configs=rows))
    total = sum(l["launches_per_step"] * l["picked_ms"] for l in layers)
    for l in layers:
        l["share_of_conv_time"] = round(l["launches_per_step"] * l["picked_ms"] / total, 4)
    layers.sort(key=lambda l: -l["share_of_conv_time"])
    res["conv_ms_per_step_at_picked"] = round(total, 3)
    res["layers"] = layers

    print(f"# {res['card']}  (mma_n={args.mma_n})  conv time per step at the picked configurations: {total:.2f} ms")
    print(f"{'shape':44s} {'n':>2s} {'share':>6s} {'pick':>9s}  " + "  ".join(f"{c:>9s}" for c in
          ("128/1", "128/2", "192/1", "256/1", "256/2")) + "   (TFLOP/s at N tile / epilogue sets, splits 1)")
    for l in layers:
        by = {(r["n_tile"], r["epilogue_sets"]): r["tflops"] for r in l["configs"] if r["splits"] == 1}
        pk = l["picked"]
        print(f"{l['shape'][:44]:44s} {l['launches_per_step']:2d} {100 * l['share_of_conv_time']:5.1f}% "
              f"{pk['n_tile']:>3d}/{pk['epilogue_sets']}/{pk['splits']:<3d}  " +
              "  ".join(f"{by.get(c, float('nan')):9.1f}" for c in ((128, 1), (128, 2), (192, 1), (256, 1), (256, 2))))
    if args.out:
        os.makedirs(os.path.dirname(os.path.abspath(args.out)), exist_ok=True)
        with open(args.out, "w") as f:
            f.write(json.dumps(res, indent=1) + "\n")


if __name__ == "__main__":
    main()
```

Baseline: 30.85.

## Write conv GEMM epilogue straight from wgmma registers via per-warp staging

Each consumer warp now runs the epilogue directly from its wgmma accumulator fragments. It uses a small swizzled per-warp shared staging buffer with ldmatrix for residual and coalesced vector stores. This replaces the old path, which dumped the full fp32 accumulator tile to shared memory, synchronised both warpgroups with named barriers, and had only some warps do the epilogue. Dropping the large accumulator buffer frees shared memory for more pipeline stages and removes the epilogue-sets variant and its tuning. The cost is more register pressure and per-warp epilogue work with narrower 16-row chunks.

```diff
diff --git a/kandinsky-2_b200/csrc/k2_api.cu b/kandinsky-2_b200/csrc/k2_api.cu
--- a/kandinsky-2_b200/csrc/k2_api.cu
+++ b/kandinsky-2_b200/csrc/k2_api.cu
@@ -26,7 +26,6 @@
 void count_launch(int n) { g_launches.fetch_add(n, std::memory_order_relaxed); }
 
 bool pdl_enabled() { return g_pdl != 0; }
-static int g_conv_epi_sets = 1;
 static int g_gn_bps = 0;
 int gn_apply_blocks_per_sm() { return g_gn_bps; }
 
@@ -132,7 +131,6 @@
   int m_tiles_phase;
   int BN, splits;
   int fuse_stats, row_groups;
-  int es;
 };
 
 static void plan_conv(int NB, int H, int W, bool any9, int kchunks, int Cout, int out_mode, bool has_workspace,
@@ -140,7 +138,6 @@
                       bool w_batched = false) {
   const int g_force_bn = (cfg && cfg[0]) ? cfg[0] : k2::g_force_bn;
   const int g_force_split = (cfg && cfg[2]) ? cfg[2] : k2::g_force_split;
-  pl.es = (cfg && cfg[3]) ? cfg[3] : k2::g_conv_epi_sets;
   choose_tile(NB, H, W, pl.TN, pl.TH, pl.TW, w_batched);
   pl.tiles_w = (W + pl.TW - 1) / pl.TW;
   pl.tiles_h = (H + pl.TH - 1) / pl.TH;
@@ -246,7 +243,6 @@
     return 0;
   }
   if (key == 10) {
-    g_conv_epi_sets = (value == 2) ? 2 : 1;
     return 0;
   }
   if (key == 11) {
@@ -374,7 +370,7 @@
     if (residual)
       K2_REQUIRE(ldr % 8 == 0 && (reinterpret_cast<uintptr_t>(residual) & 15) == 0, "conv_gemm: residual alignment");
   }
-  int rc = launch_conv_gemm(p, BN, pl.es, static_cast<cudaStream_t>(stream));
+  int rc = launch_conv_gemm(p, BN, static_cast<cudaStream_t>(stream));
   if (rc == 0) g_launches.fetch_add(1, std::memory_order_relaxed);
   if (rc == 0 && splits > 1) {
     rc = launch_splitk_finalize(p.ws, splits, p.M_total, Cout, bias, p.residual, ldr, reinterpret_cast<__half*>(out), ldo,
diff --git a/kandinsky-2_b200/csrc/k2_common.cuh b/kandinsky-2_b200/csrc/k2_common.cuh
--- a/kandinsky-2_b200/csrc/k2_common.cuh
+++ b/kandinsky-2_b200/csrc/k2_common.cuh
@@ -255,6 +255,11 @@
                : "=r"(r[0]), "=r"(r[1]), "=r"(r[2]), "=r"(r[3])
                : "r"(saddr));
 }
+__device__ __forceinline__ void stmatrix_x4(uint32_t saddr, uint32_t r0, uint32_t r1, uint32_t r2, uint32_t r3) {
+  asm volatile("stmatrix.sync.aligned.m8n8.x4.shared.b16 [%0], {%1, %2, %3, %4};" ::"r"(saddr), "r"(r0), "r"(r1), "r"(r2),
+               "r"(r3)
+               : "memory");
+}
 __device__ __forceinline__ void cp_async_16(uint32_t saddr, const void* gptr, int src_bytes) {
   asm volatile("cp.async.cg.shared.global [%0], [%1], 16, %2;" ::"r"(saddr), "l"(gptr), "r"(src_bytes) : "memory");
 }
@@ -266,6 +271,9 @@
 
 __device__ __forceinline__ void sts_v4(uint32_t saddr, uint32_t a, uint32_t b, uint32_t c, uint32_t d) {
   asm volatile("st.shared.v4.b32 [%0], {%1, %2, %3, %4};" ::"r"(saddr), "r"(a), "r"(b), "r"(c), "r"(d) : "memory");
+}
+__device__ __forceinline__ void sts_v2(uint32_t saddr, uint32_t a, uint32_t b) {
+  asm volatile("st.shared.v2.b32 [%0], {%1, %2};" ::"r"(saddr), "r"(a), "r"(b) : "memory");
 }
 __device__ __forceinline__ uint4 lds_v4(uint32_t saddr) {
   uint4 v;
diff --git a/kandinsky-2_b200/csrc/k2_conv_gemm.cu b/kandinsky-2_b200/csrc/k2_conv_gemm.cu
--- a/kandinsky-2_b200/csrc/k2_conv_gemm.cu
+++ b/kandinsky-2_b200/csrc/k2_conv_gemm.cu
@@ -10,21 +10,16 @@
 constexpr int BM = 128;
 constexpr int BK = 64;
 constexpr int A_STAGE_BYTES = BM * BK * 2;
-constexpr int ACC_PAD = 4;
-
-constexpr int EPI_STAGE_FLOATS = 32 * 33;
-constexpr int EPI_BYTES = 4 * EPI_STAGE_FLOATS * 4 + 4 * 256 * 4;
+constexpr int EPI_WARP_BYTES = 16 * 128;
 constexpr int SMEM_LIMIT = 227 * 1024;
 
-template <int BN, int ES>
+template <int BN>
 struct Cfg {
   static constexpr int B_STAGE_BYTES = BN * BK * 2;
   static constexpr int STAGE_BYTES = A_STAGE_BYTES + B_STAGE_BYTES;
-  static constexpr int BNC = (BN < 64) ? BN : (ES == 2 ? 128 : 64);
-  static_assert(ES == 1 || BN % 128 == 0, "two epilogue sets need N tiles of 128 or 256");
-  static constexpr int ACC_BYTES = BM * (BNC + ACC_PAD) * 4;
+  static constexpr int EPI_BYTES = 8 * (EPI_WARP_BYTES + BN * 4);
   static constexpr int BAR_BYTES = 256;
-  static constexpr int FIXED = ACC_BYTES + ES * EPI_BYTES + BAR_BYTES + 1024;
+  static constexpr int FIXED = EPI_BYTES + BAR_BYTES + 1024;
   static constexpr int STAGES = (SMEM_LIMIT - FIXED) / STAGE_BYTES > 6 ? 6 : (SMEM_LIMIT - FIXED) / STAGE_BYTES;
   static constexpr int SMEM_BYTES = STAGES * STAGE_BYTES + FIXED;
   static_assert(STAGES >= 2, "conv_gemm: shared memory does not hold two pipeline stages");
@@ -46,307 +41,221 @@
   n0 = tn_i * p.TN;
 }
 
-template <int N>
-__device__ __forceinline__ void acc_ld(const float* src, uint32_t (&r)[N]) {
-#pragma unroll
-  for (int v = 0; v < N / 4; ++v) {
-    const float4 t = *reinterpret_cast<const float4*>(src + 4 * v);
-    r[4 * v] = __float_as_uint(t.x);
-    r[4 * v + 1] = __float_as_uint(t.y);
-    r[4 * v + 2] = __float_as_uint(t.z);
-    r[4 * v + 3] = __float_as_uint(t.w);
-  }
-}
-
-template <int BN, int ES>
-__device__ __forceinline__ void epilogue_tile(const ConvGemmParams& p, const float* acc, int ew, int lane, int n0, int y0,
-                                              int x0, int cbase, int split, int m_idx, float* stat_smem, int es_arg,
-                                              int phase) {
-  const int es = (ES == 1) ? 0 : es_arg;
-  const int row = ew * 32 + lane;
+__device__ __forceinline__ void ldsm_x4(uint32_t (&r)[4], uint32_t saddr) {
+  asm volatile("ldmatrix.sync.aligned.m8n8.x4.shared.b16 {%0, %1, %2, %3}, [%4];"
+               : "=r"(r[0]), "=r"(r[1]), "=r"(r[2]), "=r"(r[3])
+               : "r"(saddr)
+               : "memory");
+}
+
+template <int BN>
+__device__ __forceinline__ void epilogue_warp(const ConvGemmParams& p, const float (&acc)[BN / 2], float* epi, uint32_t stg,
+                                              const float* bsm, int k, int lane, int n0, int y0, int x0, int cbase, int split,
+                                              int m_idx, int phase) {
   const int thw = p.TH * p.TW;
-  constexpr int CH = (BN >= 32) ? 32 : 16;
-  const float* arow = acc + row * (BN + ACC_PAD);
-      const int tn = row / thw;
-      const int rem = row - tn * thw;
-      const int th = rem / p.TW;
-      const int tw = rem - th * p.TW;
-      const int n = n0 + tn, y = y0 + th, x = x0 + tw;
-      const bool valid = (tn < p.TN) && (n < p.NB) && (y < p.H) && (x < p.W);
-      const long long out_row = p.up2 ? (static_cast<long long>(n) * (2 * p.H) + (2 * y + (phase >> 1))) * (2 * p.W) + (2 * x + (phase & 1))
-                                      : (static_cast<long long>(n) * p.H + y) * p.W + x;
+  auto out_row_of = [&](int row, int& n, int& y, int& x) -> long long {
+    const int tn = row / thw;
+    const int rem = row - tn * thw;
+    const int th = rem / p.TW;
+    const int tw = rem - th * p.TW;
+    n = n0 + tn;
+    y = y0 + th;
+    x = x0 + tw;
+    if (tn >= p.TN || n >= p.NB || y >= p.H || x >= p.W) return -1;
+    return p.up2 ? (static_cast<long long>(n) * (2 * p.H) + (2 * y + (phase >> 1))) * (2 * p.W) + (2 * x + (phase & 1))
+                 : (static_cast<long long>(n) * p.H + y) * p.W + x;
+  };
+  const int t4 = lane & 3, ra = lane >> 2;
+  if constexpr (BN % 64 == 0) {
+    if ((p.out_mode == 0 && p.Cout % 64 == 0) || (p.out_mode == 2 && p.Cout % 32 == 0)) {
+      int n_, y_, x_;
+      const int my_pix = static_cast<int>(out_row_of(16 * k + (lane & 15), n_, y_, x_));
+      const int sub = lane >> 3, piece = lane & 7;
+      int pix[4];
+#pragma unroll
+      for (int i = 0; i < 4; ++i) pix[i] = __shfl_sync(0xffffffffu, my_pix, 4 * i + sub);
+      const bool va = __shfl_sync(0xffffffffu, my_pix, ra) >= 0, vb = __shfl_sync(0xffffffffu, my_pix, ra + 8) >= 0;
+      auto row_addr = [&](int i) {
+        const int rr = 4 * i + sub;
+        return stg + rr * 128 + ((piece ^ (rr & 7)) << 4);
+      };
+      const int lrow = (lane & 7) + 8 * ((lane >> 3) & 1);
+      auto frag_addr = [&](int q) { return stg + lrow * 128 + (((q + (lane >> 4)) ^ (lane & 7)) << 4); };
+      if (p.out_mode == 2) {
+        float* wsb = p.ws + static_cast<long long>(split) * p.M_total * p.Cout;
+#pragma unroll
+        for (int j = 0; j < BN / 32; ++j) {
+          const int col0 = cbase + j * 32;
+          if (col0 >= p.Cout) break;
+#pragma unroll
+          for (int q = 0; q < 4; ++q) {
+#pragma unroll
+            for (int h = 0; h < 2; ++h) {
+              const int rr = ra + 8 * h;
+              const int i = 16 * j + 4 * q + 2 * h;
+              sts_v2(stg + rr * 128 + (((2 * q + (t4 >> 1)) ^ (rr & 7)) << 4) + ((t4 & 1) << 3), __float_as_uint(acc[i]),
+                     __float_as_uint(acc[i + 1]));
+            }
+          }
+          __syncwarp();
+#pragma unroll
+          for (int i = 0; i < 4; ++i) {
+            const uint4 v4 = lds_v4(row_addr(i));
+            if (pix[i] >= 0)
+              *reinterpret_cast<uint4*>(wsb + static_cast<long long>(pix[i]) * p.Cout + col0 + piece * 4) = v4;
+          }
+          __syncwarp();
+        }
+        return;
+      }
+      constexpr int NP = BN / 64;
       const int m_in = p.up2 ? m_idx - phase * p.m_tiles_phase : m_idx;
       auto part_index = [&](long long base) { return p.up2 ? base * 4 + phase : base; };
-      if constexpr (BN % 64 == 0) {
-        if ((p.out_mode == 0 && p.Cout % 64 == 0) || (p.out_mode == 2 && p.Cout % 32 == 0)) {
-          const uint32_t stage = smem_u32(stat_smem + (es * 4 + ew) * EPI_STAGE_FLOATS);
-          float* bsm = stat_smem + 4 * ES * EPI_STAGE_FLOATS + (es * 4 + ew) * 256;
-          const int my_pix = valid ? static_cast<int>(out_row) : -1;
-          const int sub = lane >> 3, piece = lane & 7;
-          int pix[8];
-#pragma unroll
-          for (int i = 0; i < 8; ++i) pix[i] = __shfl_sync(0xffffffffu, my_pix, i * 4 + sub);
-          const uint32_t own = stage + lane * 128;
-          if (p.out_mode == 2) {
-            float* wsb = p.ws + static_cast<long long>(split) * p.M_total * p.Cout;
-#pragma unroll 1
-            for (int j = 0; j < BN / 32; ++j) {
-              const int col0 = cbase + j * 32;
-              if (col0 >= p.Cout) break;
-              if constexpr (ES > 1) {
-                if ((j % ES) != es) continue;
-              }
-              uint32_t r[32];
-              acc_ld(arow + j * 32, r);
-#pragma unroll
-              for (int v = 0; v < 8; ++v)
-                sts_v4(own + ((v ^ (lane & 7)) << 4), r[v * 4], r[v * 4 + 1], r[v * 4 + 2], r[v * 4 + 3]);
-              __syncwarp();
-#pragma unroll
-              for (int i = 0; i < 8; ++i) {
-                const int rr = i * 4 + sub;
-                const uint4 v4 = lds_v4(stage + rr * 128 + ((piece ^ (rr & 7)) << 4));
-                if (pix[i] >= 0)
-                  *reinterpret_cast<uint4*>(wsb + static_cast<long long>(pix[i]) * p.Cout + col0 + piece * 4) = v4;
-              }
-              __syncwarp();
+      __half* outb = reinterpret_cast<__half*>(p.out);
+      float4 st[NP];
+      uint4 rpre[4];
+      auto load_res = [&](int j) {
+        const int c0 = cbase + j * 64;
+#pragma unroll
+        for (int i = 0; i < 4; ++i) {
+          rpre[i] = make_uint4(0u, 0u, 0u, 0u);
+          if (pix[i] >= 0 && c0 < p.Cout)
+            rpre[i] = *reinterpret_cast<const uint4*>(p.residual + static_cast<long long>(pix[i]) * p.ldr + c0 + piece * 8);
+        }
+      };
+      if (p.residual) load_res(0);
+#pragma unroll
+      for (int j = 0; j < NP; ++j) {
+        const int col0 = cbase + j * 64;
+        st[j] = make_float4(0.f, 0.f, 0.f, 0.f);
+        if (col0 >= p.Cout) continue;
+        uint32_t res[16];
+        if (p.residual) {
+#pragma unroll
+          for (int i = 0; i < 4; ++i) sts_v4(row_addr(i), rpre[i].x, rpre[i].y, rpre[i].z, rpre[i].w);
+          __syncwarp();
+#pragma unroll
+          for (int qq = 0; qq < 4; ++qq) {
+            uint32_t r4[4];
+            ldsm_x4(r4, frag_addr(2 * qq));
+#pragma unroll
+            for (int m = 0; m < 4; ++m) res[4 * qq + m] = r4[m];
+          }
+          if (j + 1 < NP) load_res(j + 1);
+          __syncwarp();
+        }
+        uint32_t o[16];
+#pragma unroll
+        for (int q = 0; q < 8; ++q) {
+#pragma unroll
+          for (int h = 0; h < 2; ++h) {
+            float f0 = acc[32 * j + 4 * q + 2 * h], f1 = acc[32 * j + 4 * q + 2 * h + 1];
+            if (p.bias) {
+              const float2 b = *reinterpret_cast<const float2*>(bsm + j * 64 + 8 * q + 2 * t4);
+              f0 += b.x;
+              f1 += b.y;
             }
-            return;
-          }
-          constexpr int NP = BN / 64;
-          if (p.bias) {
-#pragma unroll
-            for (int c = lane; c < BN; c += 32) bsm[c] = (cbase + c < p.Cout) ? __ldg(p.bias + cbase + c) : 0.f;
-            __syncwarp();
-          }
-          __half* outb = reinterpret_cast<__half*>(p.out);
-          float4 st[NP];
-          uint4 rpre[8];
-          auto load_res = [&](int jp) {
-            const int c0 = cbase + jp * 64;
-#pragma unroll
-            for (int i = 0; i < 8; ++i) {
-              rpre[i] = make_uint4(0u, 0u, 0u, 0u);
-              if (pix[i] >= 0 && c0 < p.Cout)
-                rpre[i] = *reinterpret_cast<const uint4*>(p.residual + static_cast<long long>(pix[i]) * p.ldr + c0 + piece * 8);
+            if (p.residual) {
+              const float2 t = __half22float2(*reinterpret_cast<const __half2*>(&res[2 * q + h]));
+              f0 += t.x;
+              f1 += t.y;
             }
-          };
-          if constexpr (ES == 1) {
-            if (p.residual) load_res(0);
-          }
-#pragma unroll
-          for (int jp = 0; jp < NP; ++jp) {
-            const int col0 = cbase + jp * 64;
-            st[jp] = make_float4(0.f, 0.f, 0.f, 0.f);
-            if (col0 < p.Cout && (ES == 1 || (jp % ES) == es)) {
-              if constexpr (ES > 1) {
-                if (p.residual) load_res(jp);
-              }
-              if (p.residual) {
-#pragma unroll
-                for (int i = 0; i < 8; ++i) {
-                  const int rr = i * 4 + sub;
-                  sts_v4(stage + rr * 128 + ((piece ^ (rr & 7)) << 4), rpre[i].x, rpre[i].y, rpre[i].z, rpre[i].w);
-                }
-                __syncwarp();
-              }
-              if constexpr (ES == 1) {
-                if (p.residual && jp + 1 < NP) load_res(jp + 1);
-              }
-#pragma unroll
-              for (int v = 0; v < 8; ++v) {
-                uint32_t r[8];
-                acc_ld(arow + jp * 64 + v * 8, r);
-                float f[8];
-#pragma unroll
-                for (int e = 0; e < 8; ++e) f[e] = __uint_as_float(r[e]);
-                if (p.bias) {
-                  const float4 b0 = *reinterpret_cast<const float4*>(bsm + jp * 64 + v * 8);
-                  const float4 b1 = *reinterpret_cast<const float4*>(bsm + jp * 64 + v * 8 + 4);
-                  f[0] += b0.x; f[1] += b0.y; f[2] += b0.z; f[3] += b0.w;
-                  f[4] += b1.x; f[5] += b1.y; f[6] += b1.z; f[7] += b1.w;
-                }
-                const uint32_t slot = own + ((v ^ (lane & 7)) << 4);
-                if (p.residual) {
-                  const uint4 rv = lds_v4(slot);
-                  const __half2* rh = reinterpret_cast<const __half2*>(&rv);
-#pragma unroll
-                  for (int e = 0; e < 4; ++e) {
-                    const float2 t = __half22float2(rh[e]);
-                    f[2 * e] += t.x;
-                    f[2 * e + 1] += t.y;
-                  }
-                }
-                uint32_t o[4];
-#pragma unroll
-                for (int e = 0; e < 4; ++e) {
-                  const __half2 hh = __floats2half2_rn(f[2 * e], f[2 * e + 1]);
-                  o[e] = valid ? *reinterpret_cast<const uint32_t*>(&hh) : 0u;
-                }
-                sts_v4(slot, o[0], o[1], o[2], o[3]);
-              }
-              __syncwarp();
-#pragma unroll
-              for (int i = 0; i < 8; ++i) {
-                const int rr = i * 4 + sub;
-                const uint4 v4 = lds_v4(stage + rr * 128 + ((piece ^ (rr & 7)) << 4));
-                if (pix[i] >= 0)
-                  *reinterpret_cast<uint4*>(outb + static_cast<long long>(pix[i]) * p.ldo + col0 + piece * 8) = v4;
-              }
-              if (p.gn_part) {
-                float4 h0 = make_float4(0.f, 0.f, 0.f, 0.f), h1 = make_float4(0.f, 0.f, 0.f, 0.f);
-#pragma unroll
-                for (int rr = 0; rr < 32; ++rr) {
-                  const uint32_t w = lds_u32(stage + rr * 128 + (((lane >> 2) ^ (rr & 7)) << 4) + ((lane & 3) << 2));
-                  const float2 t = __half22float2(*reinterpret_cast<const __half2*>(&w));
-                  float4& hacc = (rr < 16) ? h0 : h1;
-                  hacc.x += t.x;
-                  hacc.y = fmaf(t.x, t.x, hacc.y);
-                  hacc.z += t.y;
-                  hacc.w = fmaf(t.y, t.y, hacc.w);
-                }
-                if (p.gn_mode == 2) {
-                  const int per = p.tiles_h * p.tiles_w;
-                  const int sp = m_in % per;
-                  const int img = n0 + 2 * ew;
-                  if (2 * ew < p.TN && img < p.NB)
-                    *reinterpret_cast<float4*>(p.gn_part + part_index(static_cast<long long>(img) * per + sp) * p.Cout + col0 + 2 * lane) = h0;
-                  if (2 * ew + 1 < p.TN && img + 1 < p.NB)
-                    *reinterpret_cast<float4*>(p.gn_part + part_index(static_cast<long long>(img + 1) * per + sp) * p.Cout + col0 + 2 * lane) = h1;
-                } else {
-                  st[jp] = make_float4(h0.x + h1.x, h0.y + h1.y, h0.z + h1.z, h0.w + h1.w);
-                }
-              }
-              __syncwarp();
-            }
-          }
-          if (p.gn_part && p.gn_mode == 1) {
-            if constexpr (ES == 1) {
-              float4* mine = reinterpret_cast<float4*>(stat_smem + ew * EPI_STAGE_FLOATS);
-#pragma unroll
-              for (int jp = 0; jp < NP; ++jp) mine[jp * 32 + lane] = st[jp];
-              named_bar_sync(1, 128);
-              if (ew < NP) {
-                const int col0 = cbase + ew * 64;
-                if (col0 < p.Cout) {
-                  float4 acc = make_float4(0.f, 0.f, 0.f, 0.f);
-#pragma unroll
-                  for (int w = 0; w < 4; ++w) {
-                    const float4 t = reinterpret_cast<const float4*>(stat_smem + w * EPI_STAGE_FLOATS)[ew * 32 + lane];
-                    acc.x += t.x; acc.y += t.y; acc.z += t.z; acc.w += t.w;
-                  }
-                  *reinterpret_cast<float4*>(p.gn_part + part_index(m_in) * p.Cout + col0 + 2 * lane) = acc;
-                }
-              }
-              named_bar_sync(1, 128);
-            } else {
-              float4* mine = reinterpret_cast<float4*>(stat_smem + (es * 4 + ew) * EPI_STAGE_FLOATS);
-#pragma unroll
-              for (int jp = 0; jp < NP; ++jp) mine[jp * 32 + lane] = st[jp];
-              named_bar_sync(1 + es, 128);
-              const int jp_f = es + ew * ES;
-              if (jp_f < NP) {
-                const int col0 = cbase + jp_f * 64;
-                if (col0 < p.Cout) {
-                  float4 acc = make_float4(0.f, 0.f, 0.f, 0.f);
-#pragma unroll
-                  for (int w = 0; w < 4; ++w) {
-                    const float4 t =
-                        reinterpret_cast<const float4*>(stat_smem + (es * 4 + w) * EPI_STAGE_FLOATS)[jp_f * 32 + lane];
-                    acc.x += t.x; acc.y += t.y; acc.z += t.z; acc.w += t.w;
-                  }
-                  *reinterpret_cast<float4*>(p.gn_part + part_index(m_in) * p.Cout + col0 + 2 * lane) = acc;
-                }
-              }
-              named_bar_sync(1 + es, 128);
-            }
-          }
-          return;
-        }
-      }
-#pragma unroll 1
-      for (int j = 0; j < BN / CH; ++j) {
-        uint32_t r[CH];
-        acc_ld(arow + j * CH, r);
-        const int col0 = cbase + j * CH;
-        if (valid && col0 < p.Cout) {
-          if (p.out_mode == 2) {
-            float* w = p.ws + (static_cast<long long>(split) * p.M_total + out_row) * p.Cout + col0;
-            if (col0 + CH <= p.Cout) {
-#pragma unroll
-              for (int v = 0; v < CH / 4; ++v)
-                *reinterpret_cast<uint4*>(w + v * 4) = make_uint4(r[v * 4], r[v * 4 + 1], r[v * 4 + 2], r[v * 4 + 3]);
-            } else {
-#pragma unroll
-              for (int e = 0; e < CH; ++e)
-                if (col0 + e < p.Cout) w[e] = __uint_as_float(r[e]);
-            }
-          } else if (p.out_mode == 0) {
-            __half* orow = reinterpret_cast<__half*>(p.out) + out_row * p.ldo + col0;
-            const __half* rrow = p.residual ? p.residual + out_row * p.ldr + col0 : nullptr;
-            if (col0 + CH <= p.Cout) {
-#pragma unroll
-              for (int v = 0; v < CH / 8; ++v) {
-                float f[8];
-#pragma unroll
-                for (int e = 0; e < 8; ++e) {
-                  f[e] = __uint_as_float(r[v * 8 + e]);
-                  if (p.bias) f[e] += __ldg(p.bias + col0 + v * 8 + e);
-                }
-                if (rrow) {
-                  uint4 rv = *reinterpret_cast<const uint4*>(rrow + v * 8);
-                  const __half2* rh = reinterpret_cast<const __half2*>(&rv);
-#pragma unroll
-                  for (int e = 0; e < 4; ++e) {
-                    float2 t = __half22float2(rh[e]);
-                    f[2 * e] += t.x;
-                    f[2 * e + 1] += t.y;
-                  }
-                }
-                uint4 ov;
-                __half2* oh = reinterpret_cast<__half2*>(&ov);
-#pragma unroll
-                for (int e = 0; e < 4; ++e) oh[e] = __floats2half2_rn(f[2 * e], f[2 * e + 1]);
-                *reinterpret_cast<uint4*>(orow + v * 8) = ov;
-              }
-            } else {
-#pragma unroll
-              for (int e = 0; e < CH; ++e) {
-                if (col0 + e < p.Cout) {
-                  float f = __uint_as_float(r[e]);
-                  if (p.bias) f += __ldg(p.bias + col0 + e);
-                  if (rrow) f += __half2float(rrow[e]);
-                  orow[e] = __float2half_rn(f);
-                }
-              }
-            }
+            const __half2 hh = __floats2half2_rn(f0, f1);
+            o[2 * q + h] = (h ? vb : va) ? *reinterpret_cast<const uint32_t*>(&hh) : 0u;
+          }
+        }
+#pragma unroll
+        for (int qq = 0; qq < 4; ++qq) stmatrix_x4(frag_addr(2 * qq), o[4 * qq], o[4 * qq + 1], o[4 * qq + 2], o[4 * qq + 3]);
+        __syncwarp();
+#pragma unroll
+        for (int i = 0; i < 4; ++i) {
+          const uint4 v4 = lds_v4(row_addr(i));
+          if (pix[i] >= 0) *reinterpret_cast<uint4*>(outb + static_cast<long long>(pix[i]) * p.ldo + col0 + piece * 8) = v4;
+        }
+        if (p.gn_part) {
+          float4 hs = make_float4(0.f, 0.f, 0.f, 0.f);
+#pragma unroll
+          for (int rr = 0; rr < 16; ++rr) {
+            const uint32_t v = lds_u32(stg + rr * 128 + (((lane >> 2) ^ (rr & 7)) << 4) + ((lane & 3) << 2));
+            const float2 t = __half22float2(*reinterpret_cast<const __half2*>(&v));
+            hs.x += t.x;
+            hs.y = fmaf(t.x, t.x, hs.y);
+            hs.z += t.y;
+            hs.w = fmaf(t.y, t.y, hs.w);
+          }
+          if (p.gn_mode == 2) {
+            const int per = p.tiles_h * p.tiles_w;
+            const int sp = m_in % per;
+            const int img = n0 + k;
+            if (k < p.TN && img < p.NB)
+              *reinterpret_cast<float4*>(p.gn_part + part_index(static_cast<long long>(img) * per + sp) * p.Cout + col0 + 2 * lane) = hs;
           } else {
-            float* o = reinterpret_cast<float*>(p.out);
-#pragma unroll
-            for (int e = 0; e < CH; ++e) {
-              if (col0 + e < p.Cout) {
-                float f = __uint_as_float(r[e]);
-                if (p.bias) f += __ldg(p.bias + col0 + e);
-                o[((static_cast<long long>(n) * p.Cout + (col0 + e)) * p.H + y) * p.W + x] = f;
-              }
-            }
-          }
-        }
-      }
-}
-
-
-template <int BN, int ES>
+            st[j] = hs;
+          }
+        }
+        __syncwarp();
+      }
+      if (p.gn_part && p.gn_mode == 1) {
+        float4* sums = reinterpret_cast<float4*>(epi);
+#pragma unroll
+        for (int j = 0; j < NP; ++j) sums[k * 128 + j * 32 + lane] = st[j];
+        named_bar_sync(1, 256);
+        if (k < NP && cbase + k * 64 < p.Cout) {
+          float4 tot = make_float4(0.f, 0.f, 0.f, 0.f);
+#pragma unroll
+          for (int e = 0; e < 4; ++e) {
+            const float4 a = sums[(2 * e) * 128 + k * 32 + lane], b = sums[(2 * e + 1) * 128 + k * 32 + lane];
+            tot.x += a.x + b.x;
+            tot.y += a.y + b.y;
+            tot.z += a.z + b.z;
+            tot.w += a.w + b.w;
+          }
+          *reinterpret_cast<float4*>(p.gn_part + part_index(m_in) * p.Cout + cbase + k * 64 + 2 * lane) = tot;
+        }
+        named_bar_sync(1, 256);
+      }
+      return;
+    }
+  }
+  int n[2], y[2], x[2];
+  long long orow[2];
+#pragma unroll
+  for (int h = 0; h < 2; ++h) orow[h] = out_row_of(16 * k + ra + 8 * h, n[h], y[h], x[h]);
+#pragma unroll
+  for (int q = 0; q < BN / 8; ++q) {
+#pragma unroll
+    for (int h = 0; h < 2; ++h) {
+#pragma unroll
+      for (int e = 0; e < 2; ++e) {
+        const int col = cbase + 8 * q + 2 * t4 + e;
+        if (orow[h] < 0 || col >= p.Cout) continue;
+        float f = acc[4 * q + 2 * h + e];
+        if (p.out_mode == 2) {
+          p.ws[(static_cast<long long>(split) * p.M_total + orow[h]) * p.Cout + col] = f;
+          continue;
+        }
+        if (p.bias) f += __ldg(p.bias + col);
+        if (p.out_mode == 0) {
+          if (p.residual) f += __half2float(p.residual[orow[h] * p.ldr + col]);
+          reinterpret_cast<__half*>(p.out)[orow[h] * p.ldo + col] = __float2half_rn(f);
+        } else {
+          reinterpret_cast<float*>(p.out)[((static_cast<long long>(n[h]) * p.Cout + col) * p.H + y[h]) * p.W + x[h]] = f;
+        }
+      }
+    }
+  }
+}
+
+
+template <int BN>
 __global__ void __launch_bounds__(384, 1) conv_gemm_kernel(const __grid_constant__ ConvGemmParams p) {
-  using C = Cfg<BN, ES>;
-  constexpr int BNC = C::BNC;
+  using C = Cfg<BN>;
   constexpr int NA = BN / 2;
   extern __shared__ uint8_t smem_raw[];
   uint8_t* smem = reinterpret_cast<uint8_t*>((reinterpret_cast<uintptr_t>(smem_raw) + 1023) &
                                              ~static_cast<uintptr_t>(1023));
-  float* acc_smem = reinterpret_cast<float*>(smem + C::STAGES * C::STAGE_BYTES);
-  float* stat_smem = reinterpret_cast<float*>(smem + C::STAGES * C::STAGE_BYTES + C::ACC_BYTES);
-  uint64_t* full_bar = reinterpret_cast<uint64_t*>(smem + C::STAGES * C::STAGE_BYTES + C::ACC_BYTES + ES * EPI_BYTES);
+  float* epi = reinterpret_cast<float*>(smem + C::STAGES * C::STAGE_BYTES);
+  uint64_t* full_bar = reinterpret_cast<uint64_t*>(smem + C::STAGES * C::STAGE_BYTES + C::EPI_BYTES);
   uint64_t* empty_bar = full_bar + C::STAGES;
 
   const int warp_idx = threadIdx.x >> 5;
@@ -418,7 +327,10 @@
   } else {
     setmaxnreg_inc<232>();
     const int g = wg - 1;
-    const int w = warp_idx & 3;
+    const int k = warp_idx - 4;
+    const uint32_t stg = smem_u32(epi) + k * EPI_WARP_BYTES;
+    float* bsm = epi + 8 * EPI_WARP_BYTES / 4 + k * BN;
+    int bias_cols = -1;
     int stage = 0;
     uint32_t phase = 0;
     for (int tile = blockIdx.x; tile < total_tiles; tile += gridDim.x) {
@@ -436,9 +348,9 @@
         const uint32_t b_addr = smem_u32(smem + stage * C::STAGE_BYTES + A_STAGE_BYTES);
         wgmma_fence();
 #pragma unroll
-        for (int k = 0; k < BK / 16; ++k) {
-          const uint64_t adesc = make_wgmma_desc(a_addr) + static_cast<uint64_t>(k * 2);
-          const uint64_t bdesc = make_wgmma_desc(b_addr) + static_cast<uint64_t>(k * 2);
+        for (int ks = 0; ks < BK / 16; ++ks) {
+          const uint64_t adesc = make_wgmma_desc(a_addr) + static_cast<uint64_t>(ks * 2);
+          const uint64_t bdesc = make_wgmma_desc(b_addr) + static_cast<uint64_t>(ks * 2);
           if constexpr (BN == 256) {
             wgmma_m64n256k16(acc, adesc, bdesc, 1u);
           } else if constexpr (BN == 192) {
@@ -462,27 +374,21 @@
         }
       }
       wgmma_wait<0>();
+#pragma unroll
+      for (int i = 0; i < NA; ++i) reg_fence(acc[i]);
       if (prev_stage >= 0 && lane == 0) mbar_arrive(&empty_bar[prev_stage]);
 
       int n0, y0, x0, mphase;
       decode_m_tile(p, m_idx, n0, y0, x0, mphase);
-      const int r0 = 64 * g + 16 * w + (lane >> 2);
-      const int cq = 2 * (lane & 3);
-#pragma unroll
-      for (int pass = 0; pass < BN / BNC; ++pass) {
-        named_bar_sync(3, 256);
-#pragma unroll
-        for (int i = 0; i < NA; i += 2) {
-          if ((8 * (i >> 2)) / BNC != pass) continue;
-          const int row = r0 + 8 * ((i >> 1) & 1);
-          const int col = 8 * (i >> 2) - pass * BNC + cq;
-          *reinterpret_cast<float2*>(acc_smem + row * (BNC + ACC_PAD) + col) = make_float2(acc[i], acc[i + 1]);
-        }
-        named_bar_sync(3, 256);
-        if (ES == 2 || g == 0)
-          epilogue_tile<BNC, ES>(p, acc_smem, w, lane, n0, y0, x0, n_idx * BN + pass * BNC, split, m_idx, stat_smem, g,
-                                 mphase);
-      }
+      const int cbase = n_idx * BN;
+      if (p.bias && cbase != bias_cols) {
+        __syncwarp();
+#pragma unroll
+        for (int c = lane; c < BN; c += 32) bsm[c] = (cbase + c < p.Cout) ? __ldg(p.bias + cbase + c) : 0.f;
+        __syncwarp();
+        bias_cols = cbase;
+      }
+      epilogue_warp<BN>(p, acc, epi, stg, bsm, k, lane, n0, y0, x0, cbase, split, m_idx, mphase);
     }
   }
 }
@@ -558,18 +464,17 @@
 }
 
 
-template <int BN, int ES>
+template <int BN>
 int launch_bn(const ConvGemmParams& p, cudaStream_t stream) {
-  using C = Cfg<BN, ES>;
+  using C = Cfg<BN>;
   static bool attr_set = false;
   if (!attr_set) {
-    K2_CHECK_CUDA(cudaFuncSetAttribute(conv_gemm_kernel<BN, ES>, cudaFuncAttributeMaxDynamicSharedMemorySize,
-                                       C::SMEM_BYTES));
+    K2_CHECK_CUDA(cudaFuncSetAttribute(conv_gemm_kernel<BN>, cudaFuncAttributeMaxDynamicSharedMemorySize, C::SMEM_BYTES));
     attr_set = true;
   }
   int total = p.m_tiles * p.n_tiles * p.splits;
   int grid = total < num_sms() ? total : num_sms();
-  K2_CHECK_CUDA(launch_k(conv_gemm_kernel<BN, ES>, dim3(grid), dim3(384), C::SMEM_BYTES, stream, p));
+  K2_CHECK_CUDA(launch_k(conv_gemm_kernel<BN>, dim3(grid), dim3(384), C::SMEM_BYTES, stream, p));
   return 0;
 }
 
@@ -583,20 +488,13 @@
   return 0;
 }
 
-int launch_conv_gemm(const ConvGemmParams& p, int BN, int epilogue_sets, cudaStream_t stream) {
-  if (epilogue_sets == 2) {
-    switch (BN) {
-      case 128: return launch_bn<128, 2>(p, stream);
-      case 256: return launch_bn<256, 2>(p, stream);
-      default: break;
-    }
-  }
+int launch_conv_gemm(const ConvGemmParams& p, int BN, cudaStream_t stream) {
   switch (BN) {
-    case 16: return launch_bn<16, 1>(p, stream);
-    case 64: return launch_bn<64, 1>(p, stream);
-    case 128: return launch_bn<128, 1>(p, stream);
-    case 192: return launch_bn<192, 1>(p, stream);
-    case 256: return launch_bn<256, 1>(p, stream);
+    case 16: return launch_bn<16>(p, stream);
+    case 64: return launch_bn<64>(p, stream);
+    case 128: return launch_bn<128>(p, stream);
+    case 192: return launch_bn<192>(p, stream);
+    case 256: return launch_bn<256>(p, stream);
     default: return fail("conv_gemm: unsupported BN");
   }
 }
diff --git a/kandinsky-2_b200/csrc/k2_internal.h b/kandinsky-2_b200/csrc/k2_internal.h
--- a/kandinsky-2_b200/csrc/k2_internal.h
+++ b/kandinsky-2_b200/csrc/k2_internal.h
@@ -74,7 +74,7 @@
   int up2;
   int m_tiles_phase;
 };
-int launch_conv_gemm(const ConvGemmParams& p, int BN, int epilogue_sets, cudaStream_t stream);
+int launch_conv_gemm(const ConvGemmParams& p, int BN, cudaStream_t stream);
 int launch_splitk_finalize(const float* ws, int splits, long long M, int Cout, const float* bias, const __half* residual,
                            int ldr, __half* out, int ldo, float2* gn_part, cudaStream_t stream);
 
diff --git a/kandinsky-2_b200/kandinsky2/launch_plan.py b/kandinsky-2_b200/kandinsky2/launch_plan.py
--- a/kandinsky-2_b200/kandinsky2/launch_plan.py
+++ b/kandinsky-2_b200/kandinsky2/launch_plan.py
@@ -25,8 +25,7 @@
     best = None
     if cout > 64:
         bns = [bn0] if splits > 1 else [bn for bn in (128, 192, 256) if bn - 64 < cout or bn == bn0]
-        cands = [(bn0, 0, splits, 1)] + [(bn, 0, splits, es) for bn in bns for es in ((1,) if bn == 192 else (1, 2))
-                                        if (bn, es) != (bn0, 1)]
+        cands = [(bn0, 0, splits, 1)] + [(bn, 0, splits, 1) for bn in bns if bn != bn0]
         if 0 < m_rows <= TUNE_SMALL_M and splits == 1:
             for bn in (128, 192, 256):
                 if bn - 64 >= cout:
diff --git a/profiles/conv_layers.py b/profiles/conv_layers.py
--- a/profiles/conv_layers.py
+++ b/profiles/conv_layers.py
@@ -137,8 +137,7 @@
         cout = shp["N"]
         cfgs = []
         if cout > 64:
-            cfgs = [(bn, 0, 1, es) for bn in (128, 192, 256) if bn - 64 < cout or bn == info[0]
-                    for es in ((1,) if bn == 192 else (1, 2))]
+            cfgs = [(bn, 0, 1, 1) for bn in (128, 192, 256) if bn - 64 < cout or bn == info[0]]
         if tuple(picked_cfg) not in cfgs:
             cfgs.append(tuple(picked_cfg))
         rows = []
@@ -173,13 +172,13 @@
 
     print(f"# {res['card']}  (mma_n={args.mma_n})  conv time per step at the picked configurations: {total:.2f} ms")
     print(f"{'shape':44s} {'n':>2s} {'share':>6s} {'pick':>9s}  " + "  ".join(f"{c:>9s}" for c in
-          ("128/1", "128/2", "192/1", "256/1", "256/2")) + "   (TFLOP/s at N tile / epilogue sets, splits 1)")
+          ("128", "192", "256")) + "   (TFLOP/s at N tile, splits 1)")
     for l in layers:
         by = {(r["n_tile"], r["epilogue_sets"]): r["tflops"] for r in l["configs"] if r["splits"] == 1}
         pk = l["picked"]
         print(f"{l['shape'][:44]:44s} {l['launches_per_step']:2d} {100 * l['share_of_conv_time']:5.1f}% "
               f"{pk['n_tile']:>3d}/{pk['epilogue_sets']}/{pk['splits']:<3d}  " +
-              "  ".join(f"{by.get(c, float('nan')):9.1f}" for c in ((128, 1), (128, 2), (192, 1), (256, 1), (256, 2))))
+              "  ".join(f"{by.get(c, float('nan')):9.1f}" for c in ((128, 1), (192, 1), (256, 1))))
     if args.out:
         os.makedirs(os.path.dirname(os.path.abspath(args.out)), exist_ok=True)
         with open(args.out, "w") as f:
```

Result: faster. 32.61 (median of 6 runs) (+5.7%).
